# willis-richard/connect4

Hardware: NVIDIA B200
Metric: selfplay_positions_per_sec_at_800_sims_per_move (higher is better)
Workload: dtype fp16

## Files before the change

### connect4_b200/csrc/c4_split.cu

```cuda
#include <stdio.h>
#include <stdlib.h>
#include <string.h>
#include <unistd.h>

#include <algorithm>
#include <type_traits>
#include <chrono>
#include <mutex>
#include <thread>

#include "c4_fz.cuh"

#define SP_GMAX 16384
#define SP_GC_MAX 256
#define SP_TREE_THREADS 1024
#define SP_TREE_WARPS 31
#define SP_NB 16
#define SP_PATIENCE 4
#define SP_WATCH_SWEEPS 2048

struct SpHeader {
    unsigned ticket; unsigned pad0[31];
    int quit, abort, trees_exited, sliced; int pad2[28];
    unsigned long long prof[32];
    unsigned long long sig[16];
};
struct SpGlobal : SpHeader {
    unsigned long long ans[SP_GMAX][8];
};
__host__ __device__ constexpr size_t sp_rings_off() { return (sizeof(SpGlobal) + 255) & ~(size_t)255; }

struct SpParams {
    int n_slots;
    unsigned long long stop_games;
    unsigned long long stop_ns;
    unsigned long long slice_ns;
    const int *host_abort;
    int prof;
    int batch_ns;
    int n_tree;
    int n_net;
    unsigned ring_cap;
    int stage_nodes;
    int table_entries;
};

struct SpCtl {
    int abort, stop, tree_exited, wake;
    int status[SP_GC_MAX];
    unsigned req[SP_GC_MAX];
    const unsigned long long *watch[SP_GC_MAX];
    unsigned long long watch_tag[SP_GC_MAX];
    unsigned watch_t0[SP_GC_MAX];
    int watch_timeouts[SP_GC_MAX];
    unsigned sweep;
};

__device__ __forceinline__ unsigned ld_volu(const unsigned *p) { return *reinterpret_cast<const volatile unsigned *>(p); }
__device__ __forceinline__ unsigned long long ld_vol64(const unsigned long long *p) { return *reinterpret_cast<const volatile unsigned long long *>(p); }
__device__ __forceinline__ unsigned sp_tag(unsigned request_no) { return request_no % 16383u + 1u; }
__device__ __forceinline__ unsigned long long *sp_ring(SpGlobal *G, unsigned cap, int r)
{
    return reinterpret_cast<unsigned long long *>(reinterpret_cast<unsigned char *>(G) + sp_rings_off()) + (size_t)r * cap * 2;
}
__device__ __forceinline__ void st_volu(unsigned *p, unsigned v) { *reinterpret_cast<volatile unsigned *>(p) = v; }
#define SP_TAB_OFF ((uint32_t)((sizeof(SpCtl) + 127) & ~(size_t)127))
#define SP_TAB_STRIDE 4096u

#define SP_PROF(i, v) do { if (P.prof) atomicAdd(&G->prof[i], (unsigned long long)(v)); } while (0)

template <bool TAB>
struct SpPort {
    static constexpr int GC_MAX = SP_GC_MAX;
    static constexpr bool DEDUP = true;
    SpCtl *S;
    SpGlobal *G;
#ifdef C4_SP_STAGE_TOP
    typedef GameS GameType;
    uint32_t stage_base32;
    uint32_t stage_nodes;
    __device__ __forceinline__ void stage(GameS &g, int gl) const { g.sp32 = stage_base32 + (uint32_t)gl * stage_nodes * 32u; g.sp_nodes = stage_nodes; }
#else
    typedef typename std::conditional<TAB, GameTab<SP_TAB_OFF, SP_TAB_STRIDE>, GameNP>::type GameType;
    __device__ __forceinline__ void stage(Game &, int) const {}
#endif
    const uint32_t *memo;
    uint32_t memo_mask, memo_epoch;
    unsigned n_net, ring_cap;
    __device__ __forceinline__ int stopping() const { return ld_vol(&S->stop); }
    __device__ __forceinline__ float answer(int g, int gl, int lane) const
    {
        const unsigned tag = sp_tag(S->req[gl]);
        const unsigned long long *a = &G->ans[g][lane & 7];
        unsigned long long v = __ldcg(a);
        while (!__all_sync(FULL, (unsigned)(v >> 32) == tag)) v = ld_vol64(a);
        return (lane < 8) ? __uint_as_float((unsigned)v) : 0.f;
    }
    __device__ __forceinline__ bool impatient(int gl) const { return S->watch_timeouts[gl] >= SP_PATIENCE; }
    __device__ __forceinline__ void publish(int g, int gl, int st, bool request, u64 rc0, u64 rc1) const
    {
        unsigned tag = 0u;
        if (request) {
            const unsigned no = S->req[gl] + 1u;
            *reinterpret_cast<volatile unsigned *>(&S->req[gl]) = no;
            tag = sp_tag(no);
            S->watch_timeouts[gl] = 0;
        }
        if (st == ST_WAITMEMO) {
            S->watch[gl] = reinterpret_cast<const unsigned long long *>(memo + (size_t)memo_index(rc0, rc1, memo_mask) * 16 + 12);
            S->watch_tag[gl] = memo_pending_tag(memo_epoch, rc0, rc1);
            S->watch_t0[gl] = ld_volu(&S->sweep);
        }
        __threadfence_block();
        st_vol(&S->status[gl], st);
        if (st == ST_IDLE || st == ST_DONE) atomicAdd(&S->wake, 1);
        if (request) {
            const unsigned n = atomicAdd(&G->ticket, 1u);
            const unsigned r = n % n_net, k = n / n_net;
            const unsigned long long stamp = 1ULL + ((k / ring_cap) & 1u);
            unsigned long long *e = sp_ring(G, ring_cap, (int)r) + (size_t)(k & (ring_cap - 1u)) * 2;
            C4_DEV_ASSERT((rc0 >> 48) == 0 && (rc1 >> 48) == 0 && g < (1 << 14));
            __stcg(reinterpret_cast<ulonglong2 *>(e), make_ulonglong2(rc0 | ((unsigned long long)g << 48) | (stamp << 62),
                                                                       rc1 | ((unsigned long long)tag << 48) | (stamp << 62)));
        }
    }
};

template <bool SELFPLAY, bool TAB>
__device__ __forceinline__ void sp_tree_body(const C4Dev &dg, SpGlobal *G, const SpParams &P, SpCtl *S)
{
    const int warp = __shfl_sync(FULL, (int)(threadIdx.x >> 5), 0), lane = threadIdx.x & 31;
    const int per = P.n_slots / P.n_tree, extra = P.n_slots % P.n_tree;
    const int Gc = per + ((int)blockIdx.x < extra ? 1 : 0);
    const int g0 = (int)blockIdx.x * per + min((int)blockIdx.x, extra);

    for (int i = threadIdx.x; i < (int)(sizeof(SpCtl) / 4); i += blockDim.x) reinterpret_cast<uint32_t *>(S)[i] = 0u;
    __syncthreads();
    for (int i = threadIdx.x; i < SP_GC_MAX; i += blockDim.x) S->status[i] = (i < Gc) ? fz_entry_status(dg, g0 + i) : (int)ST_IDLE;
    if (TAB) {
        double *tab = reinterpret_cast<double *>(reinterpret_cast<unsigned char *>(S) + SP_TAB_OFF);
        for (int i = threadIdx.x; i < P.table_entries; i += blockDim.x) {
            tab[i] = dg.pbc[i]; tab[SP_TAB_STRIDE + i] = dg.sqt[i]; tab[2 * SP_TAB_STRIDE + i] = dg.rcp[i];
        }
    }
#ifdef C4_SP_STAGE_TOP
    C4Node *stage_base = reinterpret_cast<C4Node *>(reinterpret_cast<unsigned char *>(S) + ((sizeof(SpCtl) + 127) & ~(size_t)127));
    {
        const int per_game = P.stage_nodes * 2;
        for (int i = threadIdx.x; i < Gc * per_game; i += blockDim.x) {
            const int gl = i / per_game, k = i - gl * per_game;
            reinterpret_cast<uint4 *>(stage_base)[i] =
                __ldcg(reinterpret_cast<const uint4 *>(dg.pool + (size_t)(g0 + gl) * dg.blocks_per_game * C4_SLOTS) + k);
        }
    }
#endif
    __syncthreads();
    const unsigned long long t_begin = fz_globaltimer();

    if (warp == SP_TREE_WARPS) {
        for (uint32_t it = 0;; it++) {
            if (lane == 0 && (it & 7u) == 0u) {
                if (!ld_vol(&S->stop)) {
                    bool stop = false;
                    if (P.stop_games && __ldcg(&dg.ctr->games_finished) >= P.stop_games) stop = true;
                    if (P.stop_ns && fz_globaltimer() - t_begin > P.stop_ns) stop = true;
                    if (!stop && P.slice_ns && fz_globaltimer() - t_begin > P.slice_ns) { stop = true; st_vol(&G->sliced, 1); }
                    if (stop) { st_vol(&S->stop, 1); atomicAdd(&S->wake, 1); }
                }
                if ((it & 8191u) == 0u && *reinterpret_cast<const volatile int *>(P.host_abort)) st_vol(&G->abort, 1);
                if (!ld_vol(&S->abort) && ld_vol(&G->abort)) { st_vol(&S->abort, 1); atomicAdd(&S->wake, 1); }
            }
            int n_wait = 0;
            const bool look = (it & 7u) == 0u;
            for (int base = 0; base < Gc; base += 32) {
                const int i = base + lane;
                const int st = i < Gc ? ld_vol(&S->status[i]) : (int)ST_IDLE;
                const bool w = st == ST_WAIT, wm = st == ST_WAITMEMO;
                bool hit = false;
                if (w) {
                    const unsigned tag = sp_tag(ld_volu(&S->req[i]));
                    hit = (unsigned)(ld_vol64(&G->ans[g0 + i][7]) >> 32) == tag;
                    if (hit) { __threadfence_block(); st_vol(&S->status[i], FZ_ANSWERED); }
                } else if (wm && look) {
                    const bool timeout = it - S->watch_t0[i] > SP_WATCH_SWEEPS;
                    hit = *reinterpret_cast<const volatile unsigned long long *>(S->watch[i]) != S->watch_tag[i] || timeout;
                    if (hit) { if (timeout) S->watch_timeouts[i]++; __threadfence_block(); st_vol(&S->status[i], FZ_MEMOREADY); }
                }
                n_wait += __popc(__ballot_sync(FULL, w || wm));
                if (__any_sync(FULL, hit) && lane == 0) { __threadfence_block(); atomicAdd(&S->wake, 1); }
            }
            if (lane == 0) st_volu(&S->sweep, it + 1u);
            if (ld_vol(&S->tree_exited) == SP_TREE_WARPS) break;
            __nanosleep(n_wait ? 150 : 1000);
        }
        __syncwarp();
        if (lane == 0 && atomicAdd(&G->trees_exited, 1) == P.n_tree - 1) { __threadfence(); st_vol(&G->quit, 1); }
    } else {
#ifdef C4_SP_STAGE_TOP
        uint32_t stage_base32;
        asm volatile("{ .reg .u64 t; cvta.to.shared.u64 t, %1; cvt.u32.u64 %0, t; }" : "=r"(stage_base32) : "l"(stage_base));
        const SpPort<false> port{S, G, stage_base32, (uint32_t)P.stage_nodes, dg.memo, dg.memo_mask, dg.memo_epoch, (unsigned)P.n_net, P.ring_cap};
#else
        const SpPort<TAB> port{S, G, dg.memo, dg.memo_mask, dg.memo_epoch, (unsigned)P.n_net, P.ring_cap};
#endif
        int rot = (warp * 9) % Gc;
        bool idle = false;
        long long idle_t0 = 0;
        uint32_t idle_it = 0;
        long long t_run = 0, n_run = 0, t_idle = 0;
        for (;;) {
            const int seen = ld_vol(&S->wake);
            const int aborting = ld_vol(&S->abort);
            const int stop = ld_vol(&S->stop) | aborting;
            int cand = -1, n_wait = 0, n_ans = 0, n_ready = 0;
            bool cand_ans = false;
            for (int base = 0; base < Gc; base += 32) {
                const int i = base + lane;
                int idx = i + rot;
                if (idx >= Gc) idx -= Gc;
                const int s = (i < Gc) ? ld_vol(&S->status[idx]) : ST_IDLE;
                const unsigned ma = __ballot_sync(FULL, s == FZ_ANSWERED);
                const unsigned mr = __ballot_sync(FULL, s == ST_READY || s == ST_NEWROOT || s == FZ_MEMOREADY);
                const unsigned mw = __ballot_sync(FULL, s == ST_WAIT);
                n_wait += __popc(mw); n_ans += __popc(ma); n_ready += __popc(mr);
                n_ready += __popc(__ballot_sync(FULL, s == ST_WAITMEMO));
                if (ma && !cand_ans) { cand = __shfl_sync(FULL, idx, __ffs((int)ma) - 1); cand_ans = true; }
                else if (mr && cand < 0 && !stop) cand = __shfl_sync(FULL, idx, __ffs((int)mr) - 1);
            }
            if (aborting) break;
            if (cand >= 0) {
                int s = 0, ok = 0;
                if (lane == 0) {
                    s = ld_vol(&S->status[cand]);
                    if (s == FZ_ANSWERED || (!stop && (s == ST_READY || s == ST_NEWROOT || s == FZ_MEMOREADY)))
                        ok = atomicCAS(&S->status[cand], s, (int)FZ_RUNNING) == s;
                }
                ok = __shfl_sync(FULL, ok, 0);
                s = __shfl_sync(FULL, s, 0);
                if (ok) {
                    __threadfence_block();
                    const long long t_r0 = clock64();
                    if (idle) { t_idle += t_r0 - idle_t0; idle = false; }
                    fz_run_game<SELFPLAY>(dg, port, g0 + cand, cand, s, lane);
                    t_run += clock64() - t_r0; n_run++;
                    rot = cand + 1 < Gc ? cand + 1 : 0;
                }
                continue;
            }
            if (n_wait == 0 && n_ans == 0 && (stop || n_ready == 0)) break;
            if (!idle) { idle = true; idle_t0 = clock64(); idle_it = 0; }
            bool dead = false;
            while (ld_vol(&S->wake) == seen) {
                __nanosleep(idle_it < 16u ? 100 : 400);
                if ((++idle_it & 1023u) == 0u && clock64() - idle_t0 > FZ_WATCHDOG_CYCLES) {
                    if (lane == 0) { dg.ctr->engine_error = 1; st_vol(&G->abort, 1); st_vol(&S->abort, 1); atomicAdd(&S->wake, 1); }
                    dead = true;
                    break;
                }
            }
            if (dead) break;
        }
        __syncwarp();
        if (lane == 0) {
            if (P.prof) { SP_PROF(8, n_run); SP_PROF(9, t_run); SP_PROF(10, t_idle); }
            atomicAdd(&G->sig[2], (unsigned long long)t_run); atomicAdd(&G->sig[3], (unsigned long long)t_idle);
            __threadfence_block();
            atomicAdd(&S->tree_exited, 1);
        }
    }
#ifdef C4_SP_STAGE_TOP
    __syncthreads();
    {
        const int per_game = P.stage_nodes * 2;
        for (int i = threadIdx.x; i < Gc * per_game; i += blockDim.x) {
            const int gl = i / per_game, k = i - gl * per_game;
            reinterpret_cast<uint4 *>(dg.pool + (size_t)(g0 + gl) * dg.blocks_per_game * C4_SLOTS)[k] = reinterpret_cast<const uint4 *>(stage_base)[i];
        }
    }
#endif
}

struct SpNetCtl {
    int strip_nb, quit, abort, pad;
    int strip_game[SP_NB];
    unsigned strip_tag[SP_NB];
    u64 strip_c0[SP_NB], strip_c1[SP_NB];
    float ans[SP_NB][8];
};
template <int F> __host__ __device__ constexpr int sp_ctl_off(int R) { return (TcK<F>::total(R) + 15) & ~15; }
template <int F> __host__ __device__ constexpr int sp_net_smem(int R) { return sp_ctl_off<F>(R) + (int)sizeof(SpNetCtl); }

template <typename OP, int F, int EPI0, int PRODUCER, int ISSUER, bool ONE_LAUNCH>
__device__ __forceinline__ void sp_net_body(const unsigned char *__restrict__ image, int R, SpGlobal *G, C4Counters *ctr,
                                            const SpParams &P, unsigned char *smem, const unsigned tower)
{
    using K = TcK<F>;
    static_assert(K::NB <= SP_NB && K::EPI_WARPS == TC_EPI_WARPS, "strip control block / epilogue warps");
    static_assert(EPI0 % 4 == 0 || !ONE_LAUNCH, "setmaxnreg works on warpgroups");
    const int L = 1 + 2 * R;
    const int warp = __shfl_sync(FULL, (int)(threadIdx.x >> 5), 0), lane = threadIdx.x & 31;

    unsigned char *sX = smem + K::X, *sH = smem + K::H, *sW = smem + K::W;
    float *small = reinterpret_cast<float *>(smem + K::SMALL);
    const float *bias = small, *hp = small + L * F;
    float *scratch = reinterpret_cast<float *>(smem + K::scratch(R));
    uint64_t *bars = reinterpret_cast<uint64_t *>(smem + K::bars(R));
    const uint32_t b_wfull = smem_u32(bars), b_wempty = b_wfull + 8 * K::WBARS;
    const uint32_t b_accfull = b_wempty + 8 * K::WBARS, b_accempty = b_accfull + 8 * K::ACC_SLOTS;
    const uint32_t b_epi = b_accempty + 8 * K::ACC_SLOTS;
    uint32_t *tmem_slot = reinterpret_cast<uint32_t *>(bars + 2 * K::WBARS + 2 * K::ACC_SLOTS + K::T);
    SpNetCtl *S = reinterpret_cast<SpNetCtl *>(smem + sp_ctl_off<F>(R));

    for (int i = threadIdx.x; i < 2 * K::ACT_BYTES / 16; i += blockDim.x)
        reinterpret_cast<uint4 *>(sX)[i] = make_uint4(0u, 0u, 0u, 0u);
    {
        const unsigned char *src = image + (size_t)L * K::WSTAGE_BYTES;
        const int nb16 = (L * F + HEAD_FLOATS) * 4 / 16;
        for (int i = threadIdx.x; i < nb16; i += blockDim.x)
            reinterpret_cast<uint4 *>(small)[i] = reinterpret_cast<const uint4 *>(src)[i];
    }
    for (int i = threadIdx.x; i < (int)(sizeof(SpNetCtl) / 4); i += blockDim.x) reinterpret_cast<uint32_t *>(S)[i] = 0u;
    if (threadIdx.x == 0) {
        for (int i = 0; i < K::WBARS; i++) { mbar_init(b_wfull + 8 * i, 1); mbar_init(b_wempty + 8 * i, 1); }
        for (int i = 0; i < K::ACC_SLOTS; i++) { mbar_init(b_accfull + 8 * i, 1); mbar_init(b_accempty + 8 * i, K::GROUP_WARPS); }
        for (int i = 0; i < K::T; i++) mbar_init(b_epi + 8 * i, K::GROUP_WARPS);
        asm volatile("fence.mbarrier_init.release.cluster;\n" ::: "memory");
    }
    if (warp == PRODUCER) {
        asm volatile("tcgen05.alloc.cta_group::1.sync.aligned.shared::cta.b32 [%0], 512;\n" :: "r"(smem_u32(tmem_slot)) : "memory");
        asm volatile("tcgen05.relinquish_alloc_permit.cta_group::1.sync.aligned;\n" ::: "memory");
    }
    TC_PROXY_FENCE();
    TC_FENCE_BEFORE();
    __syncthreads();
    TC_FENCE_AFTER();
    const uint32_t tmem = *tmem_slot;
    if (ONE_LAUNCH) {
        if (warp >= EPI0 + 16 && (warp < (PRODUCER & ~3) || warp >= (PRODUCER & ~3) + 4)) {
            asm volatile("setmaxnreg.dec.sync.aligned.u32 24;\n");
            return;
        }
        if (warp >= (PRODUCER & ~3) && warp < (PRODUCER & ~3) + 4) {
            asm volatile("setmaxnreg.dec.sync.aligned.u32 56;\n");
            if (warp != PRODUCER && warp != ISSUER) return;
        } else {
            asm volatile("setmaxnreg.inc.sync.aligned.u32 96;\n");
        }
    }

    if (warp == PRODUCER) {
        if (lane == 0 && K::SLICED) {
            int g = 0, last[3] = {-1, -1, -1};
            bool live = true;
            for (; live; g++)
                for (int dy = 0; dy < 3 && live; dy++) {
                    if (g > 0) {
                        const uint32_t bar = b_wempty + 8 * dy, par = (uint32_t)(g - 1) & 1u;
                        for (uint32_t it = 0; !mbar_try(bar, par); it++) {
                            if (it > 4u) __nanosleep(it > 64u ? 500 : 100);
                            if ((it & 15u) == 15u && ld_vol(&S->quit)) { live = false; break; }
                        }
                        if (!live) break;
                    }
                    mbar_expect_tx(b_wfull + 8 * dy, K::WSLICE_BYTES);
                    bulk_g2s(smem_u32(sW + dy * K::WSLICE_BYTES), image + (size_t)(g % L) * K::WSTAGE_BYTES + dy * K::WSLICE_BYTES,
                             K::WSLICE_BYTES, b_wfull + 8 * dy);
                    last[dy] = g;
                }
            for (int dy = 0; dy < 3; dy++)
                if (last[dy] >= 0) mbar_wait(b_wfull + 8 * dy, (uint32_t)last[dy] & 1u);
        } else if (lane == 0) {
            int g = 0;
            bool live = true;
            for (; live; g++) {
                const int st = g % K::WSTAGES, use = g / K::WSTAGES;
                if (use > 0) {
                    const uint32_t bar = b_wempty + 8 * st, par = (uint32_t)(use - 1) & 1u;
                    for (uint32_t it = 0; !mbar_try(bar, par); it++) {
                        if (it > 4u) __nanosleep(it > 64u ? 500 : 100);
                        if ((it & 15u) == 15u && ld_vol(&S->quit)) { live = false; break; }
                    }
                    if (!live) break;
                }
                mbar_expect_tx(b_wfull + 8 * st, K::WSTAGE_BYTES);
                bulk_g2s(smem_u32(sW + st * K::WSTAGE_BYTES), image + (size_t)(g % L) * K::WSTAGE_BYTES, K::WSTAGE_BYTES,
                         b_wfull + 8 * st);
            }
            for (int i = max(0, g - K::WSTAGES); i < g; i++) mbar_wait(b_wfull + 8 * (i % K::WSTAGES), (uint32_t)(i / K::WSTAGES) & 1u);
        }
    } else if (warp == ISSUER) {
        if (lane == 0) {
            const uint32_t idesc = (1u << 4) | ((uint32_t)OP::FMT << 7) | ((uint32_t)OP::FMT << 10) |
                                   ((uint32_t)(K::NN >> 3) << 17) | ((uint32_t)(128 >> 4) << 24);
            int g = 0, c = 0;
            bool live = true;
            for (int s = 0; live; s++) {
                if (!fz_wait(b_epi, (uint32_t)(s * (L + 1)) & 1u, &S->abort)) break;
                const int nb = ld_vol(&S->strip_nb);
                if (nb == 0) break;
                const int T = (7 * nb + 15) / 16;
                for (int l = 0; l < L && live; l++, g++) {
                    const int st = g % K::WSTAGES;
                    if (!K::SLICED && !fz_wait(b_wfull + 8 * st, (uint32_t)(g / K::WSTAGES) & 1u, &S->abort)) { live = false; break; }
                    const uint32_t wbase = smem_u32(sW + st * K::WSTAGE_BYTES);
                    const uint32_t abase = smem_u32((l == 0 || (l & 1) == 0) ? sH : sX);
                    const uint64_t a_l = umma_desc(abase, K::ROWS * 16, 128);
                    const uint64_t b_l = umma_desc(wbase, K::NN * 16, 128);
                    const uint32_t ep_par = (uint32_t)(s * (L + 1) + l) & 1u;
#pragma unroll
                    for (int t = 0; t < K::T; t++, c++) {
                        if (t >= T) break;
                        if (t == 0 && !fz_wait(b_epi, ep_par, &S->abort)) { live = false; break; }
                        if (t + 1 < T && !fz_wait(b_epi + 8 * (t + 1), ep_par, &S->abort)) { live = false; break; }
                        const int slot = c % K::ACC_SLOTS, use = c / K::ACC_SLOTS;
                        if (use > 0 && !fz_wait(b_accempty + 8 * slot, (uint32_t)(use - 1) & 1u, &S->abort)) { live = false; break; }
                        TC_FENCE_AFTER();
                        const uint32_t dcol = tmem + K::ACC_COL0 + slot * K::NN;
                        const uint64_t a = a_l + (uint64_t)(128 * t);
                        if (l != 0) {
#pragma unroll
                            for (int dy = 0; dy < 3; dy++) {
                                if (K::SLICED && t == 0 && !fz_wait(b_wfull + 8 * dy, (uint32_t)g & 1u, &S->abort)) { live = false; break; }
#pragma unroll
                                for (int ks = 0; ks < K::KC / 2; ks++) {
                                    const uint64_t aa = a + 8 * dy + 2 * K::ROWS * ks, bb = b_l + (dy * K::KC + 2 * ks) * K::NN;
                                    if (dy == 0 && ks == 0) umma_f16c<0>(dcol, aa, bb, idesc); else umma_f16c<1>(dcol, aa, bb, idesc);
                                }
                                if (K::SLICED && t == T - 1) umma_commit(b_wempty + 8 * dy);
                            }
                        } else {
#pragma unroll
                            for (int dy = 0; dy < 3; dy++) {
                                if (K::SLICED && t == 0 && !fz_wait(b_wfull + 8 * dy, (uint32_t)g & 1u, &S->abort)) { live = false; break; }
                                const uint64_t aa = a + 8 * dy, bb = b_l + dy * K::STEM_KC * K::NN;
                                if (dy == 0) umma_f16c<0>(dcol, aa, bb, idesc); else umma_f16c<1>(dcol, aa, bb, idesc);
                                if (K::SLICED && t == T - 1) umma_commit(b_wempty + 8 * dy);
                            }
                        }
                        if (!live) break;
                        umma_commit(b_accfull + 8 * slot);
                    }
                    if (live && !K::SLICED) umma_commit(b_wempty + 8 * st);
                }
                if (live && !fz_wait(b_epi, (uint32_t)(s * (L + 1) + L) & 1u, &S->abort)) break;
            }
        }
    } else {
        const int e = warp - EPI0, quad = warp & 3, half = (e >> 2) % K::SLICES, group = e / K::GROUP_WARPS;
        const int et = threadIdx.x - 32 * EPI0;
        EpiCtx E;
        E.b_accfull = b_accfull; E.b_accempty = b_accempty; E.b_epi = b_epi;
        E.tmem_acc = tmem + ((uint32_t)(quad * 32) << 16) + K::ACC_COL0 + TC_CH * half;
        E.tmem_res = tmem + ((uint32_t)(quad * 32) << 16) + TC_CH * half;
        E.dst_x = sX + (size_t)(2 * half * K::ROWS + 8 + 32 * quad + lane) * 16;
        E.dst_h = sH + (size_t)(2 * half * K::ROWS + 8 + 32 * quad + lane) * 16;
        E.bias = bias; E.hp = hp;
        E.scratch = scratch + half * K::NB * 128;
        E.lane = lane; E.lm = (lane + 31) & 31; E.lp = (lane + 1) & 31; E.half = half; E.group = group;
        E.rb0 = 4 * quad + (lane >> 3); E.col8 = lane & 7;
        E.calib = nullptr;
        int c = 0;
        unsigned ring_head = 0u;
        unsigned sig_strips = 0u;
        const unsigned long long *ring = sp_ring(G, P.ring_cap, (int)tower);
        for (;;) {
            const long long t_d0 = clock64();
            long long t_work = t_d0;
            if (e == 0) {
                int k = 0;
                long long t_first = 0;
                for (uint32_t it = 1;; it++) {
                    unsigned issued = 0;
                    int q = 0;
                    if (lane == 0) {
                        const unsigned t = ld_volu(&G->ticket);
                        issued = (t + (unsigned)P.n_net - 1u - tower) / (unsigned)P.n_net;
                        q = ld_vol(&G->quit) | (ld_vol(&G->abort) << 1);
                    }
                    issued = __shfl_sync(FULL, issued, 0); q = __shfl_sync(FULL, q, 0);
                    const int avail = (int)(issued - ring_head);
                    if (q & 2) break;
                    if (avail <= 0) {
                        if (q) break;
                        if ((it & 4095u) == 0u && lane == 0 && *reinterpret_cast<const volatile int *>(P.host_abort)) st_vol(&G->abort, 1);
                        t_first = 0;
                        __nanosleep(it > 64u ? 300 : 60);
                        continue;
                    }
                    if (avail < K::NB && P.batch_ns > 0) {
                        const long long now = (long long)fz_globaltimer();
                        if (t_first == 0) t_first = now;
                        if (now - t_first < P.batch_ns) { __nanosleep(100); continue; }
                    }
                    if (P.prof) t_work = clock64();
                    k = min(avail, K::NB);
                    if (lane < k) {
                        const unsigned idx = ring_head + (unsigned)lane;
                        const unsigned long long stamp = 1ULL + ((idx / P.ring_cap) & 1u);
                        const unsigned long long *en = ring + (size_t)(idx & (P.ring_cap - 1u)) * 2;
                        unsigned long long a = 0, b = 0;
                        for (uint32_t w = 0;; w++) {
                            a = ld_vol64(en); b = ld_vol64(en + 1);
                            if ((a >> 62) == stamp && (b >> 62) == stamp) break;
                            __nanosleep(40);
                            if ((w & 255u) == 255u && ld_vol(&G->abort)) break;
                        }
                        S->strip_c0[lane] = a & 0xFFFFFFFFFFFFULL;
                        S->strip_c1[lane] = b & 0xFFFFFFFFFFFFULL;
                        S->strip_game[lane] = (int)((a >> 48) & 0x3FFFu);
                        S->strip_tag[lane] = (unsigned)((b >> 48) & 0x3FFFu);
                    }
                    ring_head += (unsigned)k;
                    sig_strips++;
                    break;
                }
                __syncwarp();
                if (lane == 0) {
                    if (k == 0) { st_vol(&S->quit, 1); atomicAdd(&G->sig[0], (unsigned long long)sig_strips); atomicAdd(&G->sig[1], (unsigned long long)ring_head); }
                    __threadfence_block();
                    st_vol(&S->strip_nb, k);
                }
            }
            EPI_BAR();
            const int nb = ld_vol(&S->strip_nb);
            const int my_game = S->strip_game[e];
            const unsigned my_tag = S->strip_tag[e];
            const long long t_d1 = clock64();
            if (nb == 0) {
                if (lane == 0 && e < K::GROUP_WARPS)
                    for (int t = 0; t < K::T; t++) mbar_arrive(b_epi + 8 * t);
                break;
            }
            const int T = (7 * nb + 15) / 16;
            E.valid_mask = 0;
            for (int t = 0; t < T; t++) {
                const int rb = 16 * t + E.rb0, b = rb / 7;
                if (E.col8 != 0 && rb - 7 * b != 0 && b < nb) E.valid_mask |= 1u << t;
            }
            for (int i = et; i < nb * 42; i += 32 * TC_EPI_WARPS) {
                const int b = i / 42, px = i - b * 42, r = px / 7, col = px - r * 7;
                const u64 a0 = S->strip_c0[b], a1 = S->strip_c1[b];
                const int bit = 7 * col + (5 - r);
                const uint32_t tomove = ((__popcll(a0 | a1) & 1) == 0) ? OP::ONE : 0u;
                const uint32_t o = (uint32_t)((a0 >> bit) & 1ULL) * OP::ONE, x = (uint32_t)((a1 >> bit) & 1ULL) * OP::ONE;
                const int row = 8 + (7 * b + 1 + r) * 8 + (col + 1);
                *reinterpret_cast<uint4 *>(sH + (size_t)row * 16) = make_uint4(tomove | (o << 16), x, 0u, 0u);
                *reinterpret_cast<uint4 *>(sH + (size_t)(K::ROWS + row) * 16) = make_uint4(0u, 0u, 0u, 0u);
            }
            TC_PROXY_FENCE();
            EPI_BAR();
            const long long t_d2 = clock64();
            if (lane == 0 && e < K::GROUP_WARPS)
                for (int t = 0; t < K::T; t++) mbar_arrive(b_epi + 8 * t);
#define SP_SKIPPED_TILES() if (lane == 0 && e < K::GROUP_WARPS) for (int t = T; t < K::T; t++) mbar_arrive(b_epi + 8 * t)
            tc_epilogue_layer<OP, F, 0>(E, 0, T, c); c += T; SP_SKIPPED_TILES();
            for (int l = 1; l < L - 1; l += 2) {
                tc_epilogue_layer<OP, F, 1>(E, l, T, c); c += T; SP_SKIPPED_TILES();
                if (l + 1 < L - 1) { tc_epilogue_layer<OP, F, 2>(E, l + 1, T, c); c += T; SP_SKIPPED_TILES(); }
            }
            tc_epilogue_layer<OP, F, 3>(E, L - 1, T, c); c += T; SP_SKIPPED_TILES();
#undef SP_SKIPPED_TILES

            EPI_BAR();
            const long long t_d3 = clock64();
            if (e < nb) {
                float *sc = scratch + e * 128;
                for (int i = lane; i < 126; i += 32) {
                    float bb = i < 42 ? hp[HO_VB] : (i < 84 ? hp[HO_PB] : hp[HO_PB + 1]);
                    float acc = sc[i];
#pragma unroll
                    for (int q = 1; q < K::SLICES; q++) acc += sc[q * K::NB * 128 + i];
                    sc[i] = leaky(acc + bb);
                }
                __syncwarp();
                float *ans = S->ans[e];
                head_tail(sc, hp, ans, lane);
                float o = (lane < 8) ? ans[lane] : 0.f;
                if (__any_sync(FULL, !isfinite(o))) {
                    o = (lane < 7) ? (1.f / 7.f) : 0.5f;
                    if (lane == 0) ctr->net_nonfinite = 1;
                }
                if (lane < 8) __stcg(&G->ans[my_game][lane], (unsigned long long)__float_as_uint(o) | ((unsigned long long)my_tag << 32));
            }
            if (P.prof && e == 0 && lane == 0) {
                SP_PROF(0, 1); SP_PROF(1, nb); SP_PROF(2, t_work - t_d0); SP_PROF(3, clock64() - t_work);
                SP_PROF(4, t_d1 - t_work); SP_PROF(5, t_d2 - t_d1); SP_PROF(6, t_d3 - t_d2); SP_PROF(7, clock64() - t_d3);
            }
        }
    }
    TC_FENCE_BEFORE();
    asm volatile("bar.sync 2, 576;\n" ::: "memory");
    if (warp == PRODUCER) {
        __syncwarp();
        asm volatile("tcgen05.dealloc.cta_group::1.sync.aligned.b32 %0, 512;\n" :: "r"(tmem) : "memory");
    }
}

template <bool SELFPLAY>
__global__ void __launch_bounds__(SP_TREE_THREADS, 1)
k_sp_tree(const C4Dev dg, SpGlobal *G, SpParams P)
{
    __shared__ SpCtl Sm;
    sp_tree_body<SELFPLAY, false>(dg, G, P, &Sm);
}
template <typename OP, int F>
__global__ void __launch_bounds__(TC_THREADS, 1)
k_sp_net(const unsigned char *__restrict__ image, int R, SpGlobal *G, C4Counters *ctr, SpParams P)
{
    extern __shared__ __align__(16) unsigned char smem[];
    sp_net_body<OP, F, 2, 0, 1, false>(image, R, G, ctr, P, smem, blockIdx.x);
}
template <typename OP, int F, bool SELFPLAY>
__global__ void __launch_bounds__(SP_TREE_THREADS, 1)
k_sp_one(const C4Dev dg, const unsigned char *__restrict__ image, int R, SpGlobal *G, SpParams P)
{
    extern __shared__ __align__(16) unsigned char smem[];
    if ((int)blockIdx.x < P.n_tree) {
#ifndef C4_SP_STAGE_TOP
        if (P.table_entries) sp_tree_body<SELFPLAY, true>(dg, G, P, reinterpret_cast<SpCtl *>(smem));
        else
#endif
        sp_tree_body<SELFPLAY, false>(dg, G, P, reinterpret_cast<SpCtl *>(smem));
    }
    else sp_net_body<OP, F, 0, 16, 17, true>(image, R, G, dg.ctr, P, smem, blockIdx.x - (unsigned)P.n_tree);
}

static int sp_sms()
{
    int dev = 0, sms = 0;
    if (cudaGetDevice(&dev) != cudaSuccess || cudaDeviceGetAttribute(&sms, cudaDevAttrMultiProcessorCount, dev) != cudaSuccess) return 0;
    return sms;
}

static int sp_net_ctas(int sms, int filters)
{
    int n = getenv("C4_SP_NET_CTAS") ? atoi(getenv("C4_SP_NET_CTAS")) : (filters == 64 ? (sms * 112 + 74) / 148 : (sms * 72 + 74) / 148);
    return std::max(1, std::min(n, sms - 1));
}

struct SpDevice {
    int *h_abort = nullptr, *d_abort = nullptr;
    SpGlobal *G = nullptr;
    cudaStream_t side = nullptr, side2 = nullptr;
    cudaEvent_t ev_a = nullptr, ev_b = nullptr;
    int coresident = 0;
    int adapt_n_net = 0;
    int last_launches = 0;
    std::mutex run;
};
static SpDevice g_sp_device[64];
static std::mutex g_sp_init;

__global__ void k_sp_probe_wait(int *flag, int *result)
{
    const unsigned long long t0 = fz_globaltimer();
    while (ld_vol(flag) == 0) {
        if (fz_globaltimer() - t0 > 200000000ULL) { *result = -1; return; }
        __nanosleep(1000);
    }
    *result = 1;
}
__global__ void k_sp_probe_set(int *flag) { st_vol(flag, 1); }

static SpDevice *sp_device()
{
    int dev = 0;
    if (cudaGetDevice(&dev) != cudaSuccess || dev < 0 || dev >= 64) return nullptr;
    SpDevice &pd = g_sp_device[dev];
    std::lock_guard<std::mutex> lock(g_sp_init);
    if (pd.G) return &pd;
    const int sms = sp_sms();
    if (sms < 8) return nullptr;
    SpGlobal *G = nullptr;
    if (cudaHostAlloc((void **)&pd.h_abort, 64, cudaHostAllocMapped) != cudaSuccess) return nullptr;
    if (cudaHostGetDevicePointer((void **)&pd.d_abort, pd.h_abort, 0) != cudaSuccess) return nullptr;
    if (cudaStreamCreateWithFlags(&pd.side, cudaStreamNonBlocking) != cudaSuccess) return nullptr;
    if (cudaStreamCreateWithFlags(&pd.side2, cudaStreamNonBlocking) != cudaSuccess) return nullptr;
    if (cudaEventCreateWithFlags(&pd.ev_a, cudaEventDisableTiming) != cudaSuccess) return nullptr;
    if (cudaEventCreateWithFlags(&pd.ev_b, cudaEventDisableTiming) != cudaSuccess) return nullptr;
    if (cudaMalloc((void **)&G, sp_rings_off() + (size_t)sms * SP_GMAX * 16) != cudaSuccess) return nullptr;
    pd.G = G;
    return &pd;
}

static bool sp_coresident(SpDevice &pd)
{
    std::lock_guard<std::mutex> lock(g_sp_init);
    if (pd.coresident != 0) return pd.coresident == 1;
    pd.coresident = -1;
    cudaFuncAttributes fa;
    if (cudaFuncGetAttributes(&fa, k_sp_probe_wait) != cudaSuccess || cudaFuncGetAttributes(&fa, k_sp_probe_set) != cudaSuccess) return false;
    int *w = reinterpret_cast<int *>(pd.G);
    if (cudaMemsetAsync(w, 0, 8, pd.side) != cudaSuccess || cudaStreamSynchronize(pd.side) != cudaSuccess) return false;
    k_sp_probe_wait<<<1, 1, 0, pd.side>>>(w, w + 1);
    k_sp_probe_set<<<1, 1, 0, pd.side2>>>(w);
    int result = 0;
    if (cudaStreamSynchronize(pd.side) != cudaSuccess || cudaStreamSynchronize(pd.side2) != cudaSuccess) return false;
    if (cudaMemcpy(&result, w + 1, sizeof(int), cudaMemcpyDeviceToHost) != cudaSuccess) return false;
    pd.coresident = result == 1 ? 1 : -1;
    if (pd.coresident < 0) fprintf(stderr, "[split] two kernels on two streams do not run side by side here (serialising tool?): one launch\n");
    return pd.coresident == 1;
}

struct SpAdapt {
    bool on = false;
    int lo = 0, hi = 0;
    double slice_ms = 25.0;
};
static void sp_adapt_bounds(SpAdapt &a, int max_games, int sms)
{
    a.lo = (sms * 40 + 74) / 148;
    a.hi = std::min((sms * 96 + 74) / 148, sms - (max_games + SP_GC_MAX - 1) / SP_GC_MAX);
}
static SpAdapt sp_adapt_config(const c4_net *net, int max_games, int sms, bool two)
{
    SpAdapt a;
    const char *e = getenv("C4_SP_ADAPT");
    if (e && atof(e) <= 0.0) return a;
    if (two || getenv("C4_SP_NET_CTAS") || net->F != 32 || max_games < 1024) return a;
    a.on = true;
    if (e && atof(e) > 1.0) a.slice_ms = atof(e);
    sp_adapt_bounds(a, max_games, sms);
    if (a.hi < a.lo) a.on = false;
    return a;
}
static int sp_adapt_next(const SpAdapt &a, int sms, int n_net, int n_tree, const unsigned long long *sig)
{
    const double NB = SP_NB, gamma = 0.145;
    const double b = sig[0] ? (double)sig[1] / (double)sig[0] : 0.0;
    const double u = b >= NB - 1.0 ? 1.0 : b * (1.0 + gamma * NB) / (NB * (1.0 + gamma * b));
    const double idle = (sig[2] + sig[3]) ? (double)sig[3] / (double)(sig[2] + sig[3]) : 0.0;
    const double rho = std::max(1e-3, n_net * u) / std::max(1e-3, n_tree * (1.0 - idle));
    double target = sms * rho / (1.0 + rho);
    if (target < n_net && idle > 0.05) target = n_net;
    target = std::max((double)n_net - 16.0, std::min((double)n_net + 16.0, target));
    int n = (int)(target / 4.0 + 0.5) * 4;
    n = std::max(a.lo, std::min(a.hi, n));
    return n;
}

extern "C" int c4_split_adapt_next(int sms, int max_games, int n_net, unsigned long long strips, unsigned long long boards,
                                   unsigned long long run_cycles, unsigned long long idle_cycles)
{
    SpAdapt a;
    a.on = true;
    sp_adapt_bounds(a, max_games, sms);
    const unsigned long long sig[4] = {strips, boards, run_cycles, idle_cycles};
    return sp_adapt_next(a, sms, n_net, std::min(sms - n_net, max_games), sig);
}

static bool c4_split_supported(const c4_net *net, int max_games)
{
    if (!net || (net->F != 32 && net->F != 64) || !net->use_tc || !net->image_tc) return false;
    if (getenv("C4_SP_DISABLE")) return false;
    const int sms = sp_sms();
    if (sms < 8 || max_games > SP_GMAX || max_games < 1) return false;
    const int n_tree = std::min(sms - sp_net_ctas(sms, net->F), max_games);
    if ((max_games + n_tree - 1) / n_tree > SP_GC_MAX) return false;
    if ((net->F == 32 ? sp_net_smem<32>(net->R) : sp_net_smem<64>(net->R)) > 227 * 1024) return false;
    const SpDevice *pd = sp_device();
    return pd != nullptr;
}

static bool sp_two_launches(SpDevice &pd)
{
    const char *want = getenv("C4_SP_LAUNCH");
    return want && !strcmp(want, "two") && sp_coresident(pd);
}

bool c4_split_eligible(const c4_net *net, int max_games, long long live_games)
{
    (void)live_games;
    const char *want = getenv("C4_ENGINE");
    if (want && (!strcmp(want, "fused") || !strcmp(want, "lockstep"))) return false;
    return c4_split_supported(net, max_games);
}

int c4_split_last_launches()
{
    SpDevice *pd = sp_device();
    return pd ? pd->last_launches : 0;
}

int c4_split_run(const C4Dev &d, const c4_net *net, int max_games, int simulations, bool selfplay,
                 unsigned long long stop_games, double stop_ms, cudaStream_t stream)
{
    const int sms = sp_sms();
    C4_REQUIRE(c4_split_supported(net, max_games), "split engine: network, pool size or device not supported");
    SpDevice &pd = *sp_device();
    std::lock_guard<std::mutex> run_lock(pd.run);
    static const bool debug = getenv("C4_FZ_DEBUG") != nullptr;
    const bool adapt_log = getenv("C4_SP_ADAPT_LOG") != nullptr;
    *reinterpret_cast<volatile int *>(pd.h_abort) = 0;
    SpParams P;
    P.n_slots = max_games;
    P.stop_games = stop_games;
    P.stop_ns = stop_ms > 0.0 ? (unsigned long long)(stop_ms * 1e6) : 0ULL;
    P.host_abort = pd.d_abort;
    P.prof = debug ? 1 : 0;
    P.batch_ns = getenv("C4_SP_BATCH_NS") ? atoi(getenv("C4_SP_BATCH_NS")) : 0;
    unsigned cap = 64;
    while ((int)cap < max_games) cap <<= 1;
    P.ring_cap = cap;
    const int smem = net->F == 32 ? sp_net_smem<32>(net->R) : sp_net_smem<64>(net->R);
    const bool two = sp_two_launches(pd);
    const SpAdapt adapt = sp_adapt_config(net, max_games, sms, two);
    int n_net = sp_net_ctas(sms, net->F);
    if (adapt.on) n_net = std::max(adapt.lo, std::min(adapt.hi, pd.adapt_n_net ? pd.adapt_n_net : (sms * 64 + 74) / 148));
    const double limit_s = getenv("C4_FZ_TIMEOUT_S") ? atof(getenv("C4_FZ_TIMEOUT_S")) : 900.0;
    const auto t_call = std::chrono::steady_clock::now();
    bool asked = false;
    pd.last_launches = 0;
    for (int slice = 0;; slice++) {
        const int n_tree = std::min(sms - n_net, max_games);
        P.n_net = n_net;
        P.n_tree = n_tree;
        P.slice_ns = 0ULL;
        if (stop_ms > 0.0) {
            const double left_ms = stop_ms - std::chrono::duration<double, std::milli>(std::chrono::steady_clock::now() - t_call).count();
            if (slice > 0 && left_ms <= 0.0) break;
            P.stop_ns = (unsigned long long)(std::max(left_ms, 0.01) * 1e6);
            if (adapt.on && left_ms > adapt.slice_ms) P.slice_ns = (unsigned long long)(adapt.slice_ms * 1e6);
        } else if (adapt.on) P.slice_ns = (unsigned long long)(adapt.slice_ms * 1e6);
        P.stage_nodes = 0;
#ifdef C4_SP_STAGE_TOP
        {
            const int gc_max = (max_games + n_tree - 1) / n_tree;
            const int avail = smem - (int)((sizeof(SpCtl) + 127) & ~(size_t)127);
            int nodes = std::min(avail / (gc_max * 32), std::min(512, d.blocks_per_game * C4_SLOTS)) & ~7;
            if (getenv("C4_SP_STAGE")) nodes = std::min(nodes, atoi(getenv("C4_SP_STAGE")) & ~7);
            P.stage_nodes = std::max(0, nodes);
        }
#endif
        P.table_entries = 0;
#ifndef C4_SP_STAGE_TOP
        {
            const bool want = getenv("C4_SP_SMEM_TABLES") ? atoi(getenv("C4_SP_SMEM_TABLES")) != 0 : true;
            const size_t need = SP_TAB_OFF + (size_t)3 * 8 * SP_TAB_STRIDE;
            if (want && !two && simulations + 2 <= (int)SP_TAB_STRIDE && need <= (size_t)smem) P.table_entries = simulations + 2;
        }
#endif
        if (two) P.stage_nodes = 0;
        C4_CUDA(cudaMemsetAsync(pd.G, 0, sp_rings_off() + (size_t)n_net * cap * 16, stream));
        if (two) {
            auto kn = net->F == 32 ? (net->fp16 ? k_sp_net<OpFP16, 32> : k_sp_net<OpBF16, 32>) : (net->fp16 ? k_sp_net<OpFP16, 64> : k_sp_net<OpBF16, 64>);
            auto kt = selfplay ? k_sp_tree<true> : k_sp_tree<false>;
            C4_CUDA(cudaFuncSetAttribute(kn, cudaFuncAttributeMaxDynamicSharedMemorySize, smem));
            {
                cudaFuncAttributes fa;
                C4_CUDA(cudaFuncGetAttributes(&fa, kn));
                C4_CUDA(cudaFuncGetAttributes(&fa, kt));
            }
            C4_CUDA(cudaEventRecord(pd.ev_a, stream));
            C4_CUDA(cudaStreamWaitEvent(pd.side, pd.ev_a, 0));
            kn<<<n_net, TC_THREADS, smem, pd.side>>>((const unsigned char *)net->image_tc, net->R, pd.G, d.ctr, P);
            C4_CUDA(cudaGetLastError());
            kt<<<n_tree, SP_TREE_THREADS, 0, stream>>>(d, pd.G, P);
            C4_CUDA(cudaGetLastError());
            C4_CUDA(cudaEventRecord(pd.ev_b, pd.side));
            C4_CUDA(cudaStreamWaitEvent(stream, pd.ev_b, 0));
            pd.last_launches += 2;
        } else {
            void (*k1)(const C4Dev, const unsigned char *, int, SpGlobal *, SpParams);
            if (net->F == 32) k1 = selfplay ? (net->fp16 ? k_sp_one<OpFP16, 32, true> : k_sp_one<OpBF16, 32, true>)
                                            : (net->fp16 ? k_sp_one<OpFP16, 32, false> : k_sp_one<OpBF16, 32, false>);
            else k1 = selfplay ? (net->fp16 ? k_sp_one<OpFP16, 64, true> : k_sp_one<OpBF16, 64, true>)
                               : (net->fp16 ? k_sp_one<OpFP16, 64, false> : k_sp_one<OpBF16, 64, false>);
            C4_CUDA(cudaFuncSetAttribute(k1, cudaFuncAttributeMaxDynamicSharedMemorySize, smem));
            k1<<<n_tree + n_net, SP_TREE_THREADS, smem, stream>>>(d, (const unsigned char *)net->image_tc, net->R, pd.G, P);
            C4_CUDA(cudaGetLastError());
            pd.last_launches += 1;
        }
        const auto t0 = std::chrono::steady_clock::now();
        for (long long it = 0;; it++) {
            cudaError_t q = cudaStreamQuery(stream);
            if (q == cudaSuccess) break;
            if (q != cudaErrorNotReady) { C4_CUDA(q); }
            const double el = std::chrono::duration<double>(std::chrono::steady_clock::now() - t_call).count();
            if (!asked && el > limit_s) { *reinterpret_cast<volatile int *>(pd.h_abort) = 1; asked = true; }
            if (asked && el > limit_s + 5.0) {
                fprintf(stderr, "[split] the launches did not end %.0f s after the abort request; giving up\n", 5.0);
                fflush(stderr);
                _exit(86);
            }
            if (it > 2000) std::this_thread::sleep_for(std::chrono::microseconds(
                std::chrono::duration<double>(std::chrono::steady_clock::now() - t0).count() > 1.0 ? 2000 : 50));
        }
        if (debug) {
            unsigned long long h[32];
            C4_CUDA(cudaMemcpy(h, pd.G->prof, sizeof(h), cudaMemcpyDeviceToHost));
            const double ns = (double)std::max(1ULL, h[0]), nr = (double)std::max(1ULL, h[8]);
            fprintf(stderr, "[split prof] %d tree CTAs + %d tower CTAs, %s | strips %llu boards/strip %.2f | tower cycles per strip: idle %.0f busy %.0f "
                            "(busy share %.2f) = claim %.0f + input %.0f + layers %.0f + heads %.0f | tree runs %llu cycles/run %.0f tree-warp idle share %.2f\n",
                    n_tree, n_net, two ? "two launches" : "one launch", h[0], h[1] / ns, h[2] / ns, h[3] / ns, h[3] / (double)std::max(1ULL, h[2] + h[3]),
                    h[4] / ns, h[5] / ns, h[6] / ns, h[7] / ns, h[8], h[9] / nr, h[10] / (double)std::max(1ULL, h[9] + h[10]));
        }
        if (!adapt.on || asked) break;
        SpHeader hd;
        C4_CUDA(cudaMemcpy(&hd, pd.G, sizeof(hd), cudaMemcpyDeviceToHost));
        if (!hd.sliced || hd.abort) break;
        const unsigned long long *sig = hd.sig;
        const int n_prev = n_net;
        n_net = sp_adapt_next(adapt, sms, n_net, n_tree, sig);
        if (adapt_log)
            fprintf(stderr, "[split adapt] slice %d: %d towers, boards/strip %.2f, tree-warp idle share %.3f -> %d towers\n", slice, n_prev,
                    sig[0] ? (double)sig[1] / (double)sig[0] : 0.0, (sig[2] + sig[3]) ? (double)sig[3] / (double)(sig[2] + sig[3]) : 0.0, n_net);
        pd.adapt_n_net = n_net;
        C4_REQUIRE(slice < (1 << 24), "split engine: did not terminate");
    }
    if (asked) { c4_set_error("split engine: host deadline passed (C4_FZ_TIMEOUT_S); the launches were aborted"); return -4; }
    return 0;
}
```

### connect4_b200/csrc/c4_tc.cuh

```cuda
#pragma once
#include <cuda_bf16.h>
#include <cuda_fp16.h>
#include <math.h>

#include "c4_common.cuh"

#define NPX 66
#define LEAKY 0.01f
#define SCRATCH_BYTES 512

#define HO_VW 0
#define HO_PW 64
#define HO_VB 192
#define HO_PB 193
#define HO_FC1B 195
#define HO_W1 196
#define HO_W2 197
#define HO_FCB 200
#define HO_FC1W 242
#define HO_POLB 284
#define HO_FCT 292
#define HO_POLW 2056
#define HEAD_FLOATS 2656

struct c4_net {
    int device;
    int F, R, n_fc;
    unsigned long long uid;
    bool fp16;
    bool use_tc;
    void *image_tc;
    void *image;
    size_t image_bytes;
    double flops;
    int scale_log2;
    float calib_max;
    c4_eval_fn ext_fn;
    void *ext_user;
    int32_t *ext_count;
};

__device__ __forceinline__ uint32_t smem_u32(const void *p) { return (uint32_t)__cvta_generic_to_shared(p); }
__device__ __forceinline__ void ldsm4(uint32_t addr, uint32_t &r0, uint32_t &r1, uint32_t &r2, uint32_t &r3)
{
    asm volatile("ldmatrix.sync.aligned.m8n8.x4.shared.b16 {%0,%1,%2,%3}, [%4];\n"
                 : "=r"(r0), "=r"(r1), "=r"(r2), "=r"(r3) : "r"(addr));
}
__device__ __forceinline__ void mma16816(float *c, const uint32_t *a, uint32_t b0, uint32_t b1)
{
    asm volatile("mma.sync.aligned.m16n8k16.row.col.f32.bf16.bf16.f32 {%0,%1,%2,%3}, {%4,%5,%6,%7}, {%8,%9}, {%0,%1,%2,%3};\n"
                 : "+f"(c[0]), "+f"(c[1]), "+f"(c[2]), "+f"(c[3])
                 : "r"(a[0]), "r"(a[1]), "r"(a[2]), "r"(a[3]), "r"(b0), "r"(b1));
}
__device__ __forceinline__ void mma16816h(float *c, const uint32_t *a, uint32_t b0, uint32_t b1)
{
    asm volatile("mma.sync.aligned.m16n8k16.row.col.f32.f16.f16.f32 {%0,%1,%2,%3}, {%4,%5,%6,%7}, {%8,%9}, {%0,%1,%2,%3};\n"
                 : "+f"(c[0]), "+f"(c[1]), "+f"(c[2]), "+f"(c[3])
                 : "r"(a[0]), "r"(a[1]), "r"(a[2]), "r"(a[3]), "r"(b0), "r"(b1));
}
__device__ __forceinline__ float leaky(float x) { return x > 0.f ? x : LEAKY * x; }

struct OpBF16 {
    static constexpr uint32_t ONE = 0x3F80u;
    static constexpr uint32_t FMT = 1u;
    __device__ static __forceinline__ void mma(float *c, const uint32_t *a, uint32_t b0, uint32_t b1) { mma16816(c, a, b0, b1); }
    __device__ static __forceinline__ uint32_t pack(float lo, float hi)
    {
        __nv_bfloat162 v = __floats2bfloat162_rn(lo, hi);
        return *reinterpret_cast<uint32_t *>(&v);
    }
    __device__ static __forceinline__ float2 unpack(uint32_t u)
    {
        return __bfloat1622float2(*reinterpret_cast<__nv_bfloat162 *>(&u));
    }
};
struct OpFP16 {
    static constexpr uint32_t ONE = 0x3C00u;
    static constexpr uint32_t FMT = 0u;
    __device__ static __forceinline__ void mma(float *c, const uint32_t *a, uint32_t b0, uint32_t b1) { mma16816h(c, a, b0, b1); }
    __device__ static __forceinline__ uint32_t pack(float lo, float hi)
    {
        __half2 v = __floats2half2_rn(lo, hi);
        return *reinterpret_cast<uint32_t *>(&v);
    }
    __device__ static __forceinline__ float2 unpack(uint32_t u) { return __half22float2(*reinterpret_cast<__half2 *>(&u)); }
};

__device__ __forceinline__ void head_tail(const float *scratch, const float *hp, float *out, int lane)
{
    float part = 0.f;
    for (int i = lane; i < 42; i += 32) {
        float a = hp[HO_FCB + i];
#pragma unroll 6
        for (int j = 0; j < 42; j++) a = fmaf(hp[HO_FCT + j * 42 + i], scratch[j], a);
        part = fmaf(hp[HO_FC1W + i], leaky(a), part);
    }
#pragma unroll
    for (int off = 16; off >= 1; off >>= 1) part += __shfl_xor_sync(0xffffffffu, part, off);
    const float value = (tanhf(part + hp[HO_FC1B]) + hp[HO_W1]) * hp[HO_W2];
    float lg[7];
#pragma unroll
    for (int k = 0; k < 7; k++) lg[k] = 0.f;
    for (int m = lane; m < 84; m += 32) {
        float xv = scratch[42 + m];
#pragma unroll
        for (int k = 0; k < 7; k++) lg[k] = fmaf(hp[HO_POLW + k * 84 + m], xv, lg[k]);
    }
#pragma unroll
    for (int k = 0; k < 7; k++) {
#pragma unroll
        for (int off = 16; off >= 1; off >>= 1) lg[k] += __shfl_xor_sync(0xffffffffu, lg[k], off);
        lg[k] += hp[HO_POLB + k];
    }
    float mx = lg[0];
#pragma unroll
    for (int k = 1; k < 7; k++) mx = fmaxf(mx, lg[k]);
    float sum = 0.f;
#pragma unroll
    for (int k = 0; k < 7; k++) { lg[k] = expf(lg[k] - mx); sum += lg[k]; }
    float mine = value;
#pragma unroll
    for (int k = 0; k < 7; k++) if (lane == k) mine = lg[k] / sum;
    if (lane < 8) out[lane] = mine;
    __syncwarp();
}

template <int F_> struct TcC;
template <> struct TcC<32> { static constexpr int F = 32, NB = 16, T = 7, ROWS = 912, WSTAGES = 3, ACC_SLOTS = 3, GROUPS = 2, EPI_WARPS = 16; static constexpr bool SLICED = false; };
template <> struct TcC<64> { static constexpr int F = 64, NB = 6, T = 3, ROWS = 400, WSTAGES = 1, ACC_SLOTS = 1, GROUPS = 1, EPI_WARPS = 16; static constexpr bool SLICED = true; };
#define TC_CH 16
#define TC_THREADS 576
#define TC_EPI_WARPS 16
template <class C_> struct TcKc : C_ {
    using C = C_;
    static constexpr int KC = C::F / 8;
    static constexpr int NN = 3 * C::F;
    static constexpr int SLICES = C::F / TC_CH;
    static constexpr int GROUP_WARPS = 4 * SLICES;
    static constexpr int ACT_BYTES = KC * C::ROWS * 16;
    static constexpr int WSTAGE_BYTES = 3 * KC * NN * 16;
    static constexpr int WSLICE_BYTES = KC * NN * 16;
    static constexpr int WBARS = C::SLICED ? 3 : C::WSTAGES;
    static constexpr int STEM_KC = C::SLICED ? KC : 2;
    static constexpr int ACC_COL0 = C::T * C::F;
    static_assert(GROUP_WARPS * C::GROUPS == C::EPI_WARPS, "epilogue warps = groups x (4 lane quadrants x channel slices)");
    static_assert(ACC_COL0 + C::ACC_SLOTS * NN <= 512, "TMEM columns");
    static_assert(16 * C::T >= 7 * C::NB && C::ROWS == 128 * C::T + 16, "strip geometry");
    static constexpr int X = 0;
    static constexpr int H = X + ACT_BYTES;
    static constexpr int W = H + ACT_BYTES;
    static constexpr int SMALL = W + C::WSTAGES * WSTAGE_BYTES;
    __host__ __device__ static constexpr int scratch(int R) { return SMALL + ((1 + 2 * R) * C::F + HEAD_FLOATS) * 4; }
    __host__ __device__ static constexpr int bars(int R) { return scratch(R) + SLICES * C::NB * 128 * 4; }
    __host__ __device__ static constexpr int total(int R) { return bars(R) + 256; }
};
template <int F_> using TcK = TcKc<TcC<F_>>;

__device__ __forceinline__ uint64_t umma_desc(uint32_t saddr, uint32_t lbo_bytes, uint32_t sbo_bytes)
{
    return (uint64_t)((saddr >> 4) & 0x3FFF) | ((uint64_t)((lbo_bytes >> 4) & 0x3FFF) << 16) |
           ((uint64_t)((sbo_bytes >> 4) & 0x3FFF) << 32) | ((uint64_t)1 << 46);
}
__device__ __forceinline__ void umma_f16(uint32_t d_tmem, uint64_t adesc, uint64_t bdesc, uint32_t idesc, uint32_t acc)
{
    asm volatile("{\n\t.reg .pred p;\n\tsetp.ne.b32 p, %4, 0;\n\t"
                 "tcgen05.mma.cta_group::1.kind::f16 [%0], %1, %2, %3, p;\n\t}\n"
                 :: "r"(d_tmem), "l"(adesc), "l"(bdesc), "r"(idesc), "r"(acc) : "memory");
}
template <int ACC>
__device__ __forceinline__ void umma_f16c(uint32_t d_tmem, uint64_t adesc, uint64_t bdesc, uint32_t idesc)
{
    asm volatile("{\n\t.reg .pred p;\n\tsetp.ne.b32 p, %4, 0;\n\t"
                 "tcgen05.mma.cta_group::1.kind::f16 [%0], %1, %2, %3, p;\n\t}\n"
                 :: "r"(d_tmem), "l"(adesc), "l"(bdesc), "r"(idesc), "n"(ACC) : "memory");
}
__device__ __forceinline__ void umma_commit(uint32_t bar)
{
    asm volatile("tcgen05.commit.cta_group::1.mbarrier::arrive::one.shared::cluster.b64 [%0];\n" :: "r"(bar) : "memory");
}
__device__ __forceinline__ void mbar_init(uint32_t bar, uint32_t count)
{
    asm volatile("mbarrier.init.shared::cta.b64 [%0], %1;\n" :: "r"(bar), "r"(count) : "memory");
}
__device__ __forceinline__ bool mbar_try(uint32_t bar, uint32_t parity)
{
    uint32_t ok;
    asm volatile("{\n\t.reg .pred p;\n\t"
                 "mbarrier.try_wait.parity.shared::cta.b64 p, [%1], %2;\n\t"
                 "selp.u32 %0, 1, 0, p;\n\t}\n" : "=r"(ok) : "r"(bar), "r"(parity) : "memory");
    return ok != 0u;
}
__device__ __forceinline__ void mbar_wait(uint32_t bar, uint32_t parity)
{
    if (mbar_try(bar, parity)) return;
    const long long t0 = clock64();
    for (uint32_t it = 1;; it++) {
        if (mbar_try(bar, parity)) return;
        if ((it & 0xfu) == 0u && clock64() - t0 > 10000000000LL) __trap();
    }
}
__device__ __forceinline__ void mbar_arrive(uint32_t bar)
{
    asm volatile("mbarrier.arrive.shared::cta.b64 _, [%0];\n" :: "r"(bar) : "memory");
}
__device__ __forceinline__ void mbar_expect_tx(uint32_t bar, uint32_t bytes)
{
    asm volatile("mbarrier.arrive.expect_tx.shared::cta.b64 _, [%0], %1;\n" :: "r"(bar), "r"(bytes) : "memory");
}
__device__ __forceinline__ void bulk_g2s(uint32_t dst, const void *src, uint32_t bytes, uint32_t bar)
{
    asm volatile("cp.async.bulk.shared::cluster.global.mbarrier::complete_tx::bytes [%0], [%1], %2, [%3];\n"
                 :: "r"(dst), "l"(src), "r"(bytes), "r"(bar) : "memory");
}
__device__ __forceinline__ void tmem_ld16(uint32_t taddr, float *r)
{
    uint32_t u[16];
    asm volatile("tcgen05.ld.sync.aligned.32x32b.x16.b32 {%0,%1,%2,%3,%4,%5,%6,%7,%8,%9,%10,%11,%12,%13,%14,%15}, [%16];\n"
                 : "=r"(u[0]), "=r"(u[1]), "=r"(u[2]), "=r"(u[3]), "=r"(u[4]), "=r"(u[5]), "=r"(u[6]), "=r"(u[7]),
                   "=r"(u[8]), "=r"(u[9]), "=r"(u[10]), "=r"(u[11]), "=r"(u[12]), "=r"(u[13]), "=r"(u[14]), "=r"(u[15])
                 : "r"(taddr) : "memory");
#pragma unroll
    for (int i = 0; i < 16; i++) r[i] = __uint_as_float(u[i]);
}
__device__ __forceinline__ void tmem_st16(uint32_t taddr, const float *r)
{
    asm volatile("tcgen05.st.sync.aligned.32x32b.x16.b32 [%0], {%1,%2,%3,%4,%5,%6,%7,%8,%9,%10,%11,%12,%13,%14,%15,%16};\n"
                 :: "r"(taddr), "r"(__float_as_uint(r[0])), "r"(__float_as_uint(r[1])), "r"(__float_as_uint(r[2])),
                    "r"(__float_as_uint(r[3])), "r"(__float_as_uint(r[4])), "r"(__float_as_uint(r[5])),
                    "r"(__float_as_uint(r[6])), "r"(__float_as_uint(r[7])), "r"(__float_as_uint(r[8])),
                    "r"(__float_as_uint(r[9])), "r"(__float_as_uint(r[10])), "r"(__float_as_uint(r[11])),
                    "r"(__float_as_uint(r[12])), "r"(__float_as_uint(r[13])), "r"(__float_as_uint(r[14])),
                    "r"(__float_as_uint(r[15])) : "memory");
}
__device__ __forceinline__ void tmem_ld8(uint32_t taddr, float *r)
{
    uint32_t u[8];
    asm volatile("tcgen05.ld.sync.aligned.32x32b.x8.b32 {%0,%1,%2,%3,%4,%5,%6,%7}, [%8];\n"
                 : "=r"(u[0]), "=r"(u[1]), "=r"(u[2]), "=r"(u[3]), "=r"(u[4]), "=r"(u[5]), "=r"(u[6]), "=r"(u[7])
                 : "r"(taddr) : "memory");
#pragma unroll
    for (int i = 0; i < 8; i++) r[i] = __uint_as_float(u[i]);
}
__device__ __forceinline__ void tmem_st8(uint32_t taddr, const float *r)
{
    asm volatile("tcgen05.st.sync.aligned.32x32b.x8.b32 [%0], {%1,%2,%3,%4,%5,%6,%7,%8};\n"
                 :: "r"(taddr), "r"(__float_as_uint(r[0])), "r"(__float_as_uint(r[1])), "r"(__float_as_uint(r[2])),
                    "r"(__float_as_uint(r[3])), "r"(__float_as_uint(r[4])), "r"(__float_as_uint(r[5])),
                    "r"(__float_as_uint(r[6])), "r"(__float_as_uint(r[7])) : "memory");
}
#define TC_FENCE_BEFORE() asm volatile("tcgen05.fence::before_thread_sync;\n" ::: "memory")
#define TC_FENCE_AFTER() asm volatile("tcgen05.fence::after_thread_sync;\n" ::: "memory")
#define TC_PROXY_FENCE() asm volatile("fence.proxy.async.shared::cta;\n" ::: "memory")
#define EPI_BAR() asm volatile("bar.sync 1, 512;\n" ::: "memory")

struct EpiCtx {
    uint32_t b_accfull, b_accempty, b_epi;
    uint32_t tmem_acc;
    uint32_t tmem_res;
    unsigned char *dst_x, *dst_h;
    const float *bias, *hp;
    float *scratch;
    uint32_t valid_mask;
    int lane, lm, lp, half, group, rb0, col8;
    unsigned *calib;
};

template <typename OP, int F, int KIND, bool CALIB = false>
__device__ __forceinline__ void tc_epilogue_layer(const EpiCtx &E, int l, int T, int c0)
{
    using K = TcK<F>;
    constexpr bool TO_RES = (KIND == 0 || KIND == 2), ADD_RES = (KIND == 2 || KIND == 3), LAST = (KIND == 3);
    unsigned char *dst = (KIND == 1) ? E.dst_h : E.dst_x;
    const float *bl = E.bias + l * F + TC_CH * E.half;
#pragma unroll 1
    for (int t = (E.group + K::GROUPS - c0 % K::GROUPS) % K::GROUPS; t < T; t += K::GROUPS) {
        const int c = c0 + t, slot = c % K::ACC_SLOTS;
        mbar_wait(E.b_accfull + 8 * slot, (uint32_t)(c / K::ACC_SLOTS) & 1u);
        TC_FENCE_AFTER();
        const uint32_t ta = E.tmem_acc + slot * K::NN;
        const uint32_t tr = E.tmem_res + F * t;
        float em[TC_CH], ez[TC_CH], ep[TC_CH], rs[TC_CH];
        tmem_ld16(ta, em);
        tmem_ld16(ta + F, ez);
        tmem_ld16(ta + 2 * F, ep);
        if (ADD_RES) tmem_ld16(tr, rs);
        asm volatile("tcgen05.wait::ld.sync.aligned;\n" ::: "memory");
        TC_FENCE_BEFORE();
        __syncwarp();
        if (E.lane == 0) mbar_arrive(E.b_accempty + 8 * slot);
        float v[TC_CH];
#pragma unroll
        for (int j = 0; j < TC_CH; j += 2) {
            float2 m1 = make_float2(__shfl_sync(0xffffffffu, em[j], E.lm), __shfl_sync(0xffffffffu, em[j + 1], E.lm));
            float2 p1 = make_float2(__shfl_sync(0xffffffffu, ep[j], E.lp), __shfl_sync(0xffffffffu, ep[j + 1], E.lp));
            float2 y = __fadd2_rn(__fadd2_rn(m1, make_float2(ez[j], ez[j + 1])), __fadd2_rn(p1, make_float2(bl[j], bl[j + 1])));
            if (ADD_RES) y = __fadd2_rn(y, make_float2(rs[j], rs[j + 1]));
            float2 z = __fmul2_rn(y, make_float2(LEAKY, LEAKY));
            v[j] = fmaxf(y.x, z.x);
            v[j + 1] = fmaxf(y.y, z.y);
        }
        const bool valid = (E.valid_mask >> t) & 1u;
        if (CALIB && valid) {
            unsigned mu = 0u;
#pragma unroll
            for (int j = 0; j < TC_CH; j++) mu = max(mu, __float_as_uint(fabsf(v[j])));
            atomicMax(E.calib, mu);
        }
        if (TO_RES) tmem_st16(tr, v);
        if (!LAST) {
            if (valid) {
                unsigned char *p = dst + (size_t)t * (128 * 16);
                *reinterpret_cast<uint4 *>(p) =
                    make_uint4(OP::pack(v[0], v[1]), OP::pack(v[2], v[3]), OP::pack(v[4], v[5]), OP::pack(v[6], v[7]));
                *reinterpret_cast<uint4 *>(p + K::ROWS * 16) =
                    make_uint4(OP::pack(v[8], v[9]), OP::pack(v[10], v[11]), OP::pack(v[12], v[13]), OP::pack(v[14], v[15]));
            }
        } else if (valid) {
            float a = 0.f, p0 = 0.f, p1 = 0.f;
#pragma unroll
            for (int j = 0; j < TC_CH; j++) {
                a = fmaf(v[j], E.hp[HO_VW + TC_CH * E.half + j], a);
                p0 = fmaf(v[j], E.hp[HO_PW + TC_CH * E.half + j], p0);
                p1 = fmaf(v[j], E.hp[HO_PW + F + TC_CH * E.half + j], p1);
            }
            const int rb = 16 * t + E.rb0, b = rb / 7;
            float *sc = E.scratch + b * 128 + (rb - 7 * b - 1) * 7 + (E.col8 - 1);
            sc[0] = a; sc[42] = p0; sc[84] = p1;
        }
        if (TO_RES) asm volatile("tcgen05.wait::st.sync.aligned;\n" ::: "memory");
        if (!LAST) TC_PROXY_FENCE();
        __syncwarp();
        if (E.lane == 0) mbar_arrive(E.b_epi + 8 * t);
    }
}

__device__ __forceinline__ void mbar_wait_idle(uint32_t bar, uint32_t parity)
{
    if (mbar_try(bar, parity)) return;
    const long long t0 = clock64();
    for (uint32_t it = 1;; it++) {
        if (mbar_try(bar, parity)) return;
        if (it > 8u) __nanosleep(it > 64u ? 256 : 32);
        if ((it & 0xfu) == 0u && clock64() - t0 > 10000000000LL) __trap();
    }
}

template <typename OP, typename K, int KIND>
__device__ __forceinline__ void tc_epilogue_layer8(const EpiCtx &E, int l, int T, int c0)
{
    constexpr int F = K::F;
    constexpr bool TO_RES = (KIND == 0 || KIND == 2), ADD_RES = (KIND == 2 || KIND == 3), LAST = (KIND == 3);
    unsigned char *dst = (KIND == 1) ? E.dst_h : E.dst_x;
    const float *bl = E.bias + l * F + TC_CH * E.half;
#pragma unroll 1
    for (int t = (E.group + K::GROUPS - c0 % K::GROUPS) % K::GROUPS; t < T; t += K::GROUPS) {
        const int c = c0 + t, slot = c % K::ACC_SLOTS;
        mbar_wait_idle(E.b_accfull + 8 * slot, (uint32_t)(c / K::ACC_SLOTS) & 1u);
        TC_FENCE_AFTER();
        const uint32_t ta = E.tmem_acc + slot * K::NN;
        const uint32_t tr = E.tmem_res + F * t;
        const bool valid = (E.valid_mask >> t) & 1u;
        float a = 0.f, p0 = 0.f, p1 = 0.f;
#pragma unroll
        for (int h0 = 0; h0 < TC_CH; h0 += 8) {
            float em[8], ez[8], ep[8], rs[8];
            tmem_ld8(ta + h0, em);
            tmem_ld8(ta + F + h0, ez);
            tmem_ld8(ta + 2 * F + h0, ep);
            if (ADD_RES) tmem_ld8(tr + h0, rs);
            asm volatile("tcgen05.wait::ld.sync.aligned;\n" ::: "memory");
            if (h0 + 8 == TC_CH) {
                TC_FENCE_BEFORE();
                __syncwarp();
                if (E.lane == 0) mbar_arrive(E.b_accempty + 8 * slot);
            }
            float v[8];
#pragma unroll
            for (int j = 0; j < 8; j += 2) {
                float2 m1 = make_float2(__shfl_sync(0xffffffffu, em[j], E.lm), __shfl_sync(0xffffffffu, em[j + 1], E.lm));
                float2 q1 = make_float2(__shfl_sync(0xffffffffu, ep[j], E.lp), __shfl_sync(0xffffffffu, ep[j + 1], E.lp));
                float2 y = __fadd2_rn(__fadd2_rn(m1, make_float2(ez[j], ez[j + 1])),
                                      __fadd2_rn(q1, make_float2(bl[h0 + j], bl[h0 + j + 1])));
                if (ADD_RES) y = __fadd2_rn(y, make_float2(rs[j], rs[j + 1]));
                float2 z = __fmul2_rn(y, make_float2(LEAKY, LEAKY));
                v[j] = fmaxf(y.x, z.x);
                v[j + 1] = fmaxf(y.y, z.y);
            }
            if (TO_RES) tmem_st8(tr + h0, v);
            if (!LAST) {
                if (valid)
                    *reinterpret_cast<uint4 *>(dst + (size_t)t * (128 * 16) + (size_t)(h0 / 8) * (K::ROWS * 16)) =
                        make_uint4(OP::pack(v[0], v[1]), OP::pack(v[2], v[3]), OP::pack(v[4], v[5]), OP::pack(v[6], v[7]));
            } else {
#pragma unroll
                for (int j = 0; j < 8; j++) {
                    a = fmaf(v[j], E.hp[HO_VW + TC_CH * E.half + h0 + j], a);
                    p0 = fmaf(v[j], E.hp[HO_PW + TC_CH * E.half + h0 + j], p0);
                    p1 = fmaf(v[j], E.hp[HO_PW + F + TC_CH * E.half + h0 + j], p1);
                }
            }
        }
        if (LAST && valid) {
            const int rb = 16 * t + E.rb0, b = rb / 7;
            float *sc = E.scratch + b * 128 + (rb - 7 * b - 1) * 7 + (E.col8 - 1);
            sc[0] = a; sc[42] = p0; sc[84] = p1;
        }
        if (TO_RES) asm volatile("tcgen05.wait::st.sync.aligned;\n" ::: "memory");
        if (!LAST) TC_PROXY_FENCE();
        __syncwarp();
        if (E.lane == 0) mbar_arrive(E.b_epi + 8 * t);
    }
}
```

Measured before the change: 459,800.

## Run two half-size 32-filter network towers per CTA with separate rings

For the 32-filter net, each network CTA now hosts two independent towers, each with 8 epilogue warps, 8-board strips, its own producer/issuer warp pair, half of the TMEM columns, its own barriers and named barrier, and its own request ring. The ticket distribution now uses n_rings = n_net × towers, and the adaptive split model gains an 8-board strip variant. The aim is lower per-strip latency and better batching with fewer boards waiting per request, in exchange for smaller MMA tiles, more shared memory and more complex warp-role logic.

New measurement: 432,300, median of 6. 6.0% lower.

```diff
diff --git a/connect4_b200/csrc/c4_split.cu b/connect4_b200/csrc/c4_split.cu
--- a/connect4_b200/csrc/c4_split.cu
+++ b/connect4_b200/csrc/c4_split.cu
@@ -15,7 +15,6 @@
 #define SP_GC_MAX 256
 #define SP_TREE_THREADS 1024
 #define SP_TREE_WARPS 31
-#define SP_NB 16
 #define SP_PATIENCE 4
 #define SP_WATCH_SWEEPS 2048
 
@@ -40,6 +39,7 @@
     int batch_ns;
     int n_tree;
     int n_net;
+    int n_rings;
     unsigned ring_cap;
     int stage_nodes;
     int table_entries;
@@ -86,7 +86,7 @@
 #endif
     const uint32_t *memo;
     uint32_t memo_mask, memo_epoch;
-    unsigned n_net, ring_cap;
+    unsigned n_rings, ring_cap;
     __device__ __forceinline__ int stopping() const { return ld_vol(&S->stop); }
     __device__ __forceinline__ float answer(int g, int gl, int lane) const
     {
@@ -116,7 +116,7 @@
         if (st == ST_IDLE || st == ST_DONE) atomicAdd(&S->wake, 1);
         if (request) {
             const unsigned n = atomicAdd(&G->ticket, 1u);
-            const unsigned r = n % n_net, k = n / n_net;
+            const unsigned r = n % n_rings, k = n / n_rings;
             const unsigned long long stamp = 1ULL + ((k / ring_cap) & 1u);
             unsigned long long *e = sp_ring(G, ring_cap, (int)r) + (size_t)(k & (ring_cap - 1u)) * 2;
             C4_DEV_ASSERT((rc0 >> 48) == 0 && (rc1 >> 48) == 0 && g < (1 << 14));
@@ -199,9 +199,9 @@
 #ifdef C4_SP_STAGE_TOP
         uint32_t stage_base32;
         asm volatile("{ .reg .u64 t; cvta.to.shared.u64 t, %1; cvt.u32.u64 %0, t; }" : "=r"(stage_base32) : "l"(stage_base));
-        const SpPort<false> port{S, G, stage_base32, (uint32_t)P.stage_nodes, dg.memo, dg.memo_mask, dg.memo_epoch, (unsigned)P.n_net, P.ring_cap};
+        const SpPort<false> port{S, G, stage_base32, (uint32_t)P.stage_nodes, dg.memo, dg.memo_mask, dg.memo_epoch, (unsigned)P.n_rings, P.ring_cap};
 #else
-        const SpPort<TAB> port{S, G, dg.memo, dg.memo_mask, dg.memo_epoch, (unsigned)P.n_net, P.ring_cap};
+        const SpPort<TAB> port{S, G, dg.memo, dg.memo_mask, dg.memo_epoch, (unsigned)P.n_rings, P.ring_cap};
 #endif
         int rot = (warp * 9) % Gc;
         bool idle = false;
@@ -280,52 +280,74 @@
 #endif
 }
 
-struct SpNetCtl {
+template <int NB> struct SpNetCtl {
     int strip_nb, quit, abort, pad;
-    int strip_game[SP_NB];
-    unsigned strip_tag[SP_NB];
-    u64 strip_c0[SP_NB], strip_c1[SP_NB];
-    float ans[SP_NB][8];
+    int strip_game[NB];
+    unsigned strip_tag[NB];
+    u64 strip_c0[NB], strip_c1[NB];
+    float ans[NB][8];
 };
-template <int F> __host__ __device__ constexpr int sp_ctl_off(int R) { return (TcK<F>::total(R) + 15) & ~15; }
-template <int F> __host__ __device__ constexpr int sp_net_smem(int R) { return sp_ctl_off<F>(R) + (int)sizeof(SpNetCtl); }
-
-template <typename OP, int F, int EPI0, int PRODUCER, int ISSUER, bool ONE_LAUNCH>
+template <int F> struct SpNet;
+template <> struct SpNet<32> { typedef TcKc<TcC32h> K; static constexpr int TOWERS = 2; };
+template <> struct SpNet<64> { typedef TcK<64> K; static constexpr int TOWERS = 1; };
+#define SP_TOWERS_MAX 2
+template <int F> struct SpMap : SpNet<F> {
+    using K = typename SpNet<F>::K;
+    static constexpr int TW = SpNet<F>::TOWERS;
+    static constexpr int THREADS = 32 * (TW * K::EPI_WARPS + 2 * TW);
+    static constexpr int TOWER_BYTES = 2 * K::ACT_BYTES + K::WSTAGES * K::WSTAGE_BYTES;
+    static constexpr int HEAD_SCRATCH = K::SLICES * K::NB * 128 * 4;
+    static constexpr int BAR_BYTES = (8 * (2 * K::WBARS + 2 * K::ACC_SLOTS + K::T) + 15) & ~15;
+    static constexpr int CTL_BYTES = ((int)sizeof(SpNetCtl<K::NB>) + 15) & ~15;
+    static constexpr int SMALL = TW * TOWER_BYTES;
+    __host__ __device__ static constexpr int X(int h) { return h * TOWER_BYTES; }
+    __host__ __device__ static constexpr int scratch(int R, int h) { return SMALL + ((1 + 2 * R) * K::F + HEAD_FLOATS) * 4 + h * HEAD_SCRATCH; }
+    __host__ __device__ static constexpr int bars(int R, int h) { return scratch(R, TW) + h * BAR_BYTES; }
+    __host__ __device__ static constexpr int tmem_slot(int R) { return bars(R, TW); }
+    __host__ __device__ static constexpr int ctl(int R, int h) { return tmem_slot(R) + 16 + h * CTL_BYTES; }
+    __host__ __device__ static constexpr int total(int R) { return ctl(R, TW); }
+    static_assert(TW * K::EPI_WARPS == 16, "16 epilogue warps at 96 registers (setmaxnreg budget of the one-launch form)");
+    static_assert(K::ACC_COL0 + K::ACC_SLOTS * K::NN <= 512 / TW, "TMEM columns of a tower");
+    static_assert(TW <= SP_TOWERS_MAX && 1 + TW < 16, "rings / named barriers");
+};
+template <int F> __host__ __device__ constexpr int sp_net_smem(int R) { return SpMap<F>::total(R); }
+static_assert(SpMap<32>::total(3) <= 201104, "shared memory of a 32-filter tower CTA");
+
+template <typename OP, int F, int EPI0, int PRODUCER, bool ONE_LAUNCH>
 __device__ __forceinline__ void sp_net_body(const unsigned char *__restrict__ image, int R, SpGlobal *G, C4Counters *ctr,
-                                            const SpParams &P, unsigned char *smem, const unsigned tower)
-{
-    using K = TcK<F>;
-    static_assert(K::NB <= SP_NB && K::EPI_WARPS == TC_EPI_WARPS, "strip control block / epilogue warps");
+                                            const SpParams &P, unsigned char *smem, const unsigned cta)
+{
+    using M = SpMap<F>;
+    using K = typename M::K;
+    constexpr int TW = M::TW, EW = K::EPI_WARPS;
     static_assert(EPI0 % 4 == 0 || !ONE_LAUNCH, "setmaxnreg works on warpgroups");
+    static_assert(PRODUCER % 4 == 0 && (PRODUCER >= EPI0 + 16 || PRODUCER + 2 * TW <= EPI0), "producer / issuer warps");
     const int L = 1 + 2 * R;
     const int warp = __shfl_sync(FULL, (int)(threadIdx.x >> 5), 0), lane = threadIdx.x & 31;
-
-    unsigned char *sX = smem + K::X, *sH = smem + K::H, *sW = smem + K::W;
-    float *small = reinterpret_cast<float *>(smem + K::SMALL);
+    float *small = reinterpret_cast<float *>(smem + M::SMALL);
     const float *bias = small, *hp = small + L * F;
-    float *scratch = reinterpret_cast<float *>(smem + K::scratch(R));
-    uint64_t *bars = reinterpret_cast<uint64_t *>(smem + K::bars(R));
-    const uint32_t b_wfull = smem_u32(bars), b_wempty = b_wfull + 8 * K::WBARS;
-    const uint32_t b_accfull = b_wempty + 8 * K::WBARS, b_accempty = b_accfull + 8 * K::ACC_SLOTS;
-    const uint32_t b_epi = b_accempty + 8 * K::ACC_SLOTS;
-    uint32_t *tmem_slot = reinterpret_cast<uint32_t *>(bars + 2 * K::WBARS + 2 * K::ACC_SLOTS + K::T);
-    SpNetCtl *S = reinterpret_cast<SpNetCtl *>(smem + sp_ctl_off<F>(R));
-
-    for (int i = threadIdx.x; i < 2 * K::ACT_BYTES / 16; i += blockDim.x)
-        reinterpret_cast<uint4 *>(sX)[i] = make_uint4(0u, 0u, 0u, 0u);
+
+    for (int h = 0; h < TW; h++)
+        for (int i = threadIdx.x; i < 2 * K::ACT_BYTES / 16; i += blockDim.x)
+            reinterpret_cast<uint4 *>(smem + M::X(h))[i] = make_uint4(0u, 0u, 0u, 0u);
     {
         const unsigned char *src = image + (size_t)L * K::WSTAGE_BYTES;
         const int nb16 = (L * F + HEAD_FLOATS) * 4 / 16;
         for (int i = threadIdx.x; i < nb16; i += blockDim.x)
             reinterpret_cast<uint4 *>(small)[i] = reinterpret_cast<const uint4 *>(src)[i];
     }
-    for (int i = threadIdx.x; i < (int)(sizeof(SpNetCtl) / 4); i += blockDim.x) reinterpret_cast<uint32_t *>(S)[i] = 0u;
+    for (int i = threadIdx.x; i < TW * M::CTL_BYTES / 4; i += blockDim.x) reinterpret_cast<uint32_t *>(smem + M::ctl(R, 0))[i] = 0u;
     if (threadIdx.x == 0) {
-        for (int i = 0; i < K::WBARS; i++) { mbar_init(b_wfull + 8 * i, 1); mbar_init(b_wempty + 8 * i, 1); }
-        for (int i = 0; i < K::ACC_SLOTS; i++) { mbar_init(b_accfull + 8 * i, 1); mbar_init(b_accempty + 8 * i, K::GROUP_WARPS); }
-        for (int i = 0; i < K::T; i++) mbar_init(b_epi + 8 * i, K::GROUP_WARPS);
+        for (int h = 0; h < TW; h++) {
+            const uint32_t b0 = smem_u32(smem + M::bars(R, h));
+            const uint32_t b_wf = b0, b_we = b_wf + 8 * K::WBARS, b_af = b_we + 8 * K::WBARS, b_ae = b_af + 8 * K::ACC_SLOTS;
+            for (int i = 0; i < K::WBARS; i++) { mbar_init(b_wf + 8 * i, 1); mbar_init(b_we + 8 * i, 1); }
+            for (int i = 0; i < K::ACC_SLOTS; i++) { mbar_init(b_af + 8 * i, 1); mbar_init(b_ae + 8 * i, K::GROUP_WARPS); }
+            for (int i = 0; i < K::T; i++) mbar_init(b_ae + 8 * K::ACC_SLOTS + 8 * i, K::GROUP_WARPS);
+        }
         asm volatile("fence.mbarrier_init.release.cluster;\n" ::: "memory");
     }
+    uint32_t *tmem_slot = reinterpret_cast<uint32_t *>(smem + M::tmem_slot(R));
     if (warp == PRODUCER) {
         asm volatile("tcgen05.alloc.cta_group::1.sync.aligned.shared::cta.b32 [%0], 512;\n" :: "r"(smem_u32(tmem_slot)) : "memory");
         asm volatile("tcgen05.relinquish_alloc_permit.cta_group::1.sync.aligned;\n" ::: "memory");
@@ -334,21 +356,31 @@
     TC_FENCE_BEFORE();
     __syncthreads();
     TC_FENCE_AFTER();
-    const uint32_t tmem = *tmem_slot;
-    if (ONE_LAUNCH) {
-        if (warp >= EPI0 + 16 && (warp < (PRODUCER & ~3) || warp >= (PRODUCER & ~3) + 4)) {
-            asm volatile("setmaxnreg.dec.sync.aligned.u32 24;\n");
-            return;
-        }
-        if (warp >= (PRODUCER & ~3) && warp < (PRODUCER & ~3) + 4) {
-            asm volatile("setmaxnreg.dec.sync.aligned.u32 56;\n");
-            if (warp != PRODUCER && warp != ISSUER) return;
-        } else {
-            asm volatile("setmaxnreg.inc.sync.aligned.u32 96;\n");
-        }
-    }
-
-    if (warp == PRODUCER) {
+    const uint32_t tmem0 = *tmem_slot;
+    const bool epi = warp >= EPI0 && warp < EPI0 + 16;
+    const int h = TW == 1 ? 0 : epi ? (warp - EPI0) / EW : (warp - PRODUCER) >> 1;
+    const unsigned tower = (unsigned)TW * cta + (unsigned)h;
+    unsigned char *sX = smem + M::X(h), *sH = sX + K::ACT_BYTES, *sW = sH + K::ACT_BYTES;
+    float *scratch = reinterpret_cast<float *>(smem + M::scratch(R, h));
+    const uint32_t b_wfull = smem_u32(smem + M::bars(R, h)), b_wempty = b_wfull + 8 * K::WBARS;
+    const uint32_t b_accfull = b_wempty + 8 * K::WBARS, b_accempty = b_accfull + 8 * K::ACC_SLOTS;
+    const uint32_t b_epi = b_accempty + 8 * K::ACC_SLOTS;
+    SpNetCtl<K::NB> *S = reinterpret_cast<SpNetCtl<K::NB> *>(smem + M::ctl(R, h));
+    const uint32_t tmem = tmem0 + (uint32_t)(h * (512 / TW));
+#define SP_EPI_BAR() do { if (TW == 1 || h == 0) asm volatile("bar.sync 1, %0;\n" :: "n"(32 * EW) : "memory"); \
+                        else asm volatile("bar.sync 2, %0;\n" :: "n"(32 * EW) : "memory"); } while (0)
+
+    if (ONE_LAUNCH && !epi && (warp < PRODUCER || warp >= PRODUCER + 4)) {
+        asm volatile("setmaxnreg.dec.sync.aligned.u32 24;\n");
+        return;
+    }
+
+    if (!epi) {
+      if (ONE_LAUNCH) {
+        asm volatile("setmaxnreg.dec.sync.aligned.u32 56;\n");
+        if (warp >= PRODUCER + 2 * TW) return;
+      }
+      if (((warp - PRODUCER) & 1) == 0) {
         if (lane == 0 && K::SLICED) {
             int g = 0, last[3] = {-1, -1, -1};
             bool live = true;
@@ -388,7 +420,7 @@
             }
             for (int i = max(0, g - K::WSTAGES); i < g; i++) mbar_wait(b_wfull + 8 * (i % K::WSTAGES), (uint32_t)(i / K::WSTAGES) & 1u);
         }
-    } else if (warp == ISSUER) {
+      } else {
         if (lane == 0) {
             const uint32_t idesc = (1u << 4) | ((uint32_t)OP::FMT << 7) | ((uint32_t)OP::FMT << 10) |
                                    ((uint32_t)(K::NN >> 3) << 17) | ((uint32_t)(128 >> 4) << 24);
@@ -434,8 +466,10 @@
                                 if (K::SLICED && t == 0 && !fz_wait(b_wfull + 8 * dy, (uint32_t)g & 1u, &S->abort)) { live = false; break; }
                                 const uint64_t aa = a + 8 * dy, bb = b_l + dy * K::STEM_KC * K::NN;
                                 if (dy == 0) umma_f16c<0>(dcol, aa, bb, idesc); else umma_f16c<1>(dcol, aa, bb, idesc);
-                                if (K::SLICED && t == T - 1) umma_commit(b_wempty + 8 * dy);
+                                if (K::SLICED && K::STEM_KC == K::KC && t == T - 1) umma_commit(b_wempty + 8 * dy);
                             }
+                            if (live && K::SLICED && K::STEM_KC != K::KC && t == T - 1)
+                                for (int dy = 0; dy < 3; dy++) umma_commit(b_wempty + 8 * dy);
                         }
                         if (!live) break;
                         umma_commit(b_accfull + 8 * slot);
@@ -445,9 +479,11 @@
                 if (live && !fz_wait(b_epi, (uint32_t)(s * (L + 1) + L) & 1u, &S->abort)) break;
             }
         }
+      }
     } else {
-        const int e = warp - EPI0, quad = warp & 3, half = (e >> 2) % K::SLICES, group = e / K::GROUP_WARPS;
-        const int et = threadIdx.x - 32 * EPI0;
+        if (ONE_LAUNCH) asm volatile("setmaxnreg.inc.sync.aligned.u32 96;\n");
+        const int e = warp - EPI0 - h * EW, quad = warp & 3, half = (e >> 2) % K::SLICES, group = e / K::GROUP_WARPS;
+        const int et = threadIdx.x - 32 * (EPI0 + h * EW);
         EpiCtx E;
         E.b_accfull = b_accfull; E.b_accempty = b_accempty; E.b_epi = b_epi;
         E.tmem_acc = tmem + ((uint32_t)(quad * 32) << 16) + K::ACC_COL0 + TC_CH * half;
@@ -474,7 +510,7 @@
                     int q = 0;
                     if (lane == 0) {
                         const unsigned t = ld_volu(&G->ticket);
-                        issued = (t + (unsigned)P.n_net - 1u - tower) / (unsigned)P.n_net;
+                        issued = (t + (unsigned)P.n_rings - 1u - tower) / (unsigned)P.n_rings;
                         q = ld_vol(&G->quit) | (ld_vol(&G->abort) << 1);
                     }
                     issued = __shfl_sync(FULL, issued, 0); q = __shfl_sync(FULL, q, 0);
@@ -521,10 +557,10 @@
                     st_vol(&S->strip_nb, k);
                 }
             }
-            EPI_BAR();
+            SP_EPI_BAR();
             const int nb = ld_vol(&S->strip_nb);
-            const int my_game = S->strip_game[e];
-            const unsigned my_tag = S->strip_tag[e];
+            const int my_game = e < K::NB ? S->strip_game[e] : 0;
+            const unsigned my_tag = e < K::NB ? S->strip_tag[e] : 0u;
             const long long t_d1 = clock64();
             if (nb == 0) {
                 if (lane == 0 && e < K::GROUP_WARPS)
@@ -537,7 +573,7 @@
                 const int rb = 16 * t + E.rb0, b = rb / 7;
                 if (E.col8 != 0 && rb - 7 * b != 0 && b < nb) E.valid_mask |= 1u << t;
             }
-            for (int i = et; i < nb * 42; i += 32 * TC_EPI_WARPS) {
+            for (int i = et; i < nb * 42; i += 32 * EW) {
                 const int b = i / 42, px = i - b * 42, r = px / 7, col = px - r * 7;
                 const u64 a0 = S->strip_c0[b], a1 = S->strip_c1[b];
                 const int bit = 7 * col + (5 - r);
@@ -548,20 +584,20 @@
                 *reinterpret_cast<uint4 *>(sH + (size_t)(K::ROWS + row) * 16) = make_uint4(0u, 0u, 0u, 0u);
             }
             TC_PROXY_FENCE();
-            EPI_BAR();
+            SP_EPI_BAR();
             const long long t_d2 = clock64();
             if (lane == 0 && e < K::GROUP_WARPS)
                 for (int t = 0; t < K::T; t++) mbar_arrive(b_epi + 8 * t);
 #define SP_SKIPPED_TILES() if (lane == 0 && e < K::GROUP_WARPS) for (int t = T; t < K::T; t++) mbar_arrive(b_epi + 8 * t)
-            tc_epilogue_layer<OP, F, 0>(E, 0, T, c); c += T; SP_SKIPPED_TILES();
+            tc_epilogue_layer<OP, F, 0, false, K>(E, 0, T, c); c += T; SP_SKIPPED_TILES();
             for (int l = 1; l < L - 1; l += 2) {
-                tc_epilogue_layer<OP, F, 1>(E, l, T, c); c += T; SP_SKIPPED_TILES();
-                if (l + 1 < L - 1) { tc_epilogue_layer<OP, F, 2>(E, l + 1, T, c); c += T; SP_SKIPPED_TILES(); }
-            }
-            tc_epilogue_layer<OP, F, 3>(E, L - 1, T, c); c += T; SP_SKIPPED_TILES();
+                tc_epilogue_layer<OP, F, 1, false, K>(E, l, T, c); c += T; SP_SKIPPED_TILES();
+                if (l + 1 < L - 1) { tc_epilogue_layer<OP, F, 2, false, K>(E, l + 1, T, c); c += T; SP_SKIPPED_TILES(); }
+            }
+            tc_epilogue_layer<OP, F, 3, false, K>(E, L - 1, T, c); c += T; SP_SKIPPED_TILES();
 #undef SP_SKIPPED_TILES
 
-            EPI_BAR();
+            SP_EPI_BAR();
             const long long t_d3 = clock64();
             if (e < nb) {
                 float *sc = scratch + e * 128;
@@ -588,11 +624,12 @@
             }
         }
     }
+#undef SP_EPI_BAR
     TC_FENCE_BEFORE();
-    asm volatile("bar.sync 2, 576;\n" ::: "memory");
+    asm volatile("bar.sync %0, %1;\n" :: "n"(1 + TW), "n"(M::THREADS) : "memory");
     if (warp == PRODUCER) {
         __syncwarp();
-        asm volatile("tcgen05.dealloc.cta_group::1.sync.aligned.b32 %0, 512;\n" :: "r"(tmem) : "memory");
+        asm volatile("tcgen05.dealloc.cta_group::1.sync.aligned.b32 %0, 512;\n" :: "r"(tmem0) : "memory");
     }
 }
 
@@ -604,11 +641,11 @@
     sp_tree_body<SELFPLAY, false>(dg, G, P, &Sm);
 }
 template <typename OP, int F>
-__global__ void __launch_bounds__(TC_THREADS, 1)
+__global__ void __launch_bounds__(SpMap<F>::THREADS, 1)
 k_sp_net(const unsigned char *__restrict__ image, int R, SpGlobal *G, C4Counters *ctr, SpParams P)
 {
     extern __shared__ __align__(16) unsigned char smem[];
-    sp_net_body<OP, F, 2, 0, 1, false>(image, R, G, ctr, P, smem, blockIdx.x);
+    sp_net_body<OP, F, 2 * SpMap<F>::TW, 0, false>(image, R, G, ctr, P, smem, blockIdx.x);
 }
 template <typename OP, int F, bool SELFPLAY>
 __global__ void __launch_bounds__(SP_TREE_THREADS, 1)
@@ -622,7 +659,7 @@
 #endif
         sp_tree_body<SELFPLAY, false>(dg, G, P, reinterpret_cast<SpCtl *>(smem));
     }
-    else sp_net_body<OP, F, 0, 16, 17, true>(image, R, G, dg.ctr, P, smem, blockIdx.x - (unsigned)P.n_tree);
+    else sp_net_body<OP, F, 0, 16, true>(image, R, G, dg.ctr, P, smem, blockIdx.x - (unsigned)P.n_tree);
 }
 
 static int sp_sms()
@@ -678,7 +715,7 @@
     if (cudaStreamCreateWithFlags(&pd.side2, cudaStreamNonBlocking) != cudaSuccess) return nullptr;
     if (cudaEventCreateWithFlags(&pd.ev_a, cudaEventDisableTiming) != cudaSuccess) return nullptr;
     if (cudaEventCreateWithFlags(&pd.ev_b, cudaEventDisableTiming) != cudaSuccess) return nullptr;
-    if (cudaMalloc((void **)&G, sp_rings_off() + (size_t)sms * SP_GMAX * 16) != cudaSuccess) return nullptr;
+    if (cudaMalloc((void **)&G, sp_rings_off() + (size_t)SP_TOWERS_MAX * sms * SP_GMAX * 16) != cudaSuccess) return nullptr;
     pd.G = G;
     return &pd;
 }
@@ -724,11 +761,14 @@
     if (a.hi < a.lo) a.on = false;
     return a;
 }
-static int sp_adapt_next(const SpAdapt &a, int sms, int n_net, int n_tree, const unsigned long long *sig)
-{
-    const double NB = SP_NB, gamma = 0.145;
+struct SpStripModel { double nb, gamma; };
+static constexpr SpStripModel SP_STRIPS_8 = {8.0, 0.30};
+static constexpr SpStripModel SP_STRIPS_16 = {16.0, 0.145};
+static int sp_adapt_next(const SpAdapt &a, const SpStripModel &m, int sms, int n_net, int n_tree, const unsigned long long *sig)
+{
+    const double NB = m.nb, gamma = m.gamma;
     const double b = sig[0] ? (double)sig[1] / (double)sig[0] : 0.0;
-    const double u = b >= NB - 1.0 ? 1.0 : b * (1.0 + gamma * NB) / (NB * (1.0 + gamma * b));
+    const double u = b >= NB * (15.0 / 16.0) ? 1.0 : b * (1.0 + gamma * NB) / (NB * (1.0 + gamma * b));
     const double idle = (sig[2] + sig[3]) ? (double)sig[3] / (double)(sig[2] + sig[3]) : 0.0;
     const double rho = std::max(1e-3, n_net * u) / std::max(1e-3, n_tree * (1.0 - idle));
     double target = sms * rho / (1.0 + rho);
@@ -746,7 +786,7 @@
     a.on = true;
     sp_adapt_bounds(a, max_games, sms);
     const unsigned long long sig[4] = {strips, boards, run_cycles, idle_cycles};
-    return sp_adapt_next(a, sms, n_net, std::min(sms - n_net, max_games), sig);
+    return sp_adapt_next(a, SP_STRIPS_16, sms, n_net, std::min(sms - n_net, max_games), sig);
 }
 
 static bool c4_split_supported(const c4_net *net, int max_games)
@@ -814,6 +854,7 @@
     for (int slice = 0;; slice++) {
         const int n_tree = std::min(sms - n_net, max_games);
         P.n_net = n_net;
+        P.n_rings = n_net * (net->F == 32 ? SpNet<32>::TOWERS : SpNet<64>::TOWERS);
         P.n_tree = n_tree;
         P.slice_ns = 0ULL;
         if (stop_ms > 0.0) {
@@ -841,7 +882,7 @@
         }
 #endif
         if (two) P.stage_nodes = 0;
-        C4_CUDA(cudaMemsetAsync(pd.G, 0, sp_rings_off() + (size_t)n_net * cap * 16, stream));
+        C4_CUDA(cudaMemsetAsync(pd.G, 0, sp_rings_off() + (size_t)P.n_rings * cap * 16, stream));
         if (two) {
             auto kn = net->F == 32 ? (net->fp16 ? k_sp_net<OpFP16, 32> : k_sp_net<OpBF16, 32>) : (net->fp16 ? k_sp_net<OpFP16, 64> : k_sp_net<OpBF16, 64>);
             auto kt = selfplay ? k_sp_tree<true> : k_sp_tree<false>;
@@ -853,7 +894,7 @@
             }
             C4_CUDA(cudaEventRecord(pd.ev_a, stream));
             C4_CUDA(cudaStreamWaitEvent(pd.side, pd.ev_a, 0));
-            kn<<<n_net, TC_THREADS, smem, pd.side>>>((const unsigned char *)net->image_tc, net->R, pd.G, d.ctr, P);
+            kn<<<n_net, net->F == 32 ? SpMap<32>::THREADS : SpMap<64>::THREADS, smem, pd.side>>>((const unsigned char *)net->image_tc, net->R, pd.G, d.ctr, P);
             C4_CUDA(cudaGetLastError());
             kt<<<n_tree, SP_TREE_THREADS, 0, stream>>>(d, pd.G, P);
             C4_CUDA(cudaGetLastError());
@@ -890,9 +931,9 @@
             unsigned long long h[32];
             C4_CUDA(cudaMemcpy(h, pd.G->prof, sizeof(h), cudaMemcpyDeviceToHost));
             const double ns = (double)std::max(1ULL, h[0]), nr = (double)std::max(1ULL, h[8]);
-            fprintf(stderr, "[split prof] %d tree CTAs + %d tower CTAs, %s | strips %llu boards/strip %.2f | tower cycles per strip: idle %.0f busy %.0f "
+            fprintf(stderr, "[split prof] %d tree CTAs + %d tower CTAs (%d towers), %s | strips %llu boards/strip %.2f | tower cycles per strip: idle %.0f busy %.0f "
                             "(busy share %.2f) = claim %.0f + input %.0f + layers %.0f + heads %.0f | tree runs %llu cycles/run %.0f tree-warp idle share %.2f\n",
-                    n_tree, n_net, two ? "two launches" : "one launch", h[0], h[1] / ns, h[2] / ns, h[3] / ns, h[3] / (double)std::max(1ULL, h[2] + h[3]),
+                    n_tree, n_net, P.n_rings, two ? "two launches" : "one launch", h[0], h[1] / ns, h[2] / ns, h[3] / ns, h[3] / (double)std::max(1ULL, h[2] + h[3]),
                     h[4] / ns, h[5] / ns, h[6] / ns, h[7] / ns, h[8], h[9] / nr, h[10] / (double)std::max(1ULL, h[9] + h[10]));
         }
         if (!adapt.on || asked) break;
@@ -901,7 +942,7 @@
         if (!hd.sliced || hd.abort) break;
         const unsigned long long *sig = hd.sig;
         const int n_prev = n_net;
-        n_net = sp_adapt_next(adapt, sms, n_net, n_tree, sig);
+        n_net = sp_adapt_next(adapt, SP_STRIPS_8, sms, n_net, n_tree, sig);
         if (adapt_log)
             fprintf(stderr, "[split adapt] slice %d: %d towers, boards/strip %.2f, tree-warp idle share %.3f -> %d towers\n", slice, n_prev,
                     sig[0] ? (double)sig[1] / (double)sig[0] : 0.0, (sig[2] + sig[3]) ? (double)sig[3] / (double)(sig[2] + sig[3]) : 0.0, n_net);
diff --git a/connect4_b200/csrc/c4_tc.cuh b/connect4_b200/csrc/c4_tc.cuh
--- a/connect4_b200/csrc/c4_tc.cuh
+++ b/connect4_b200/csrc/c4_tc.cuh
@@ -128,6 +128,7 @@
 template <int F_> struct TcC;
 template <> struct TcC<32> { static constexpr int F = 32, NB = 16, T = 7, ROWS = 912, WSTAGES = 3, ACC_SLOTS = 3, GROUPS = 2, EPI_WARPS = 16; static constexpr bool SLICED = false; };
 template <> struct TcC<64> { static constexpr int F = 64, NB = 6, T = 3, ROWS = 400, WSTAGES = 1, ACC_SLOTS = 1, GROUPS = 1, EPI_WARPS = 16; static constexpr bool SLICED = true; };
+struct TcC32h { static constexpr int F = 32, NB = 8, T = 4, ROWS = 528, WSTAGES = 1, ACC_SLOTS = 1, GROUPS = 1, EPI_WARPS = 8; static constexpr bool SLICED = true; };
 #define TC_CH 16
 #define TC_THREADS 576
 #define TC_EPI_WARPS 16
@@ -141,7 +142,7 @@
     static constexpr int WSTAGE_BYTES = 3 * KC * NN * 16;
     static constexpr int WSLICE_BYTES = KC * NN * 16;
     static constexpr int WBARS = C::SLICED ? 3 : C::WSTAGES;
-    static constexpr int STEM_KC = C::SLICED ? KC : 2;
+    static constexpr int STEM_KC = C::F == 32 ? 2 : KC;
     static constexpr int ACC_COL0 = C::T * C::F;
     static_assert(GROUP_WARPS * C::GROUPS == C::EPI_WARPS, "epilogue warps = groups x (4 lane quadrants x channel slices)");
     static_assert(ACC_COL0 + C::ACC_SLOTS * NN <= 512, "TMEM columns");
@@ -265,10 +266,10 @@
     unsigned *calib;
 };
 
-template <typename OP, int F, int KIND, bool CALIB = false>
+template <typename OP, int F, int KIND, bool CALIB = false, class K = TcK<F>>
 __device__ __forceinline__ void tc_epilogue_layer(const EpiCtx &E, int l, int T, int c0)
 {
-    using K = TcK<F>;
+    static_assert(K::F == F, "geometry of another filter count");
     constexpr bool TO_RES = (KIND == 0 || KIND == 2), ADD_RES = (KIND == 2 || KIND == 3), LAST = (KIND == 3);
     unsigned char *dst = (KIND == 1) ? E.dst_h : E.dst_x;
     const float *bl = E.bias + l * F + TC_CH * E.half;
```
